# volcengine/veScale

Hardware: AMD Instinct MI355X
Metric: tokens/sec (whole node) Llama-3-8B veScale-FSDP (higher is better)
Workload: dtype bf16; 1 GPU; model=llama3_8b, global_batch=4, seq_len=8192, parallelism=fsdp1, activation_checkpointing=False, hipgraph=True

## Files before the change

### vescale_amd/ops/csrc/attention_bwd.hip

```cpp
#include "common.h"

#define FA_D 128
#define FA_BLK 64
#define FA_THREADS 256
#define FA_PAD 8

typedef float fa_floatx4 __attribute__((ext_vector_type(4)));
typedef short fa_shortx8 __attribute__((ext_vector_type(8)));

extern "C" __global__ void __launch_bounds__(256)
fa_bwd_preprocess(const unsigned short* __restrict__ dout,
                  const unsigned short* __restrict__ o,
                  float* __restrict__ delta, int64_t rows) {
  const int sub = threadIdx.x & 15;
  int64_t row = (int64_t)blockIdx.x * 16 + (threadIdx.x >> 4);
  const int64_t stride = (int64_t)gridDim.x * 16;
  for (; row < rows; row += stride) {
    const unsigned short* pd = dout + row * FA_D + sub * 8;
    const unsigned short* po = o + row * FA_D + sub * 8;
    fa_shortx8 a = *reinterpret_cast<const fa_shortx8*>(pd);
    fa_shortx8 b = *reinterpret_cast<const fa_shortx8*>(po);
    float s = 0.f;
#pragma unroll
    for (int j = 0; j < 8; ++j)
      s += bf16_to_f32((unsigned short)a[j]) * bf16_to_f32((unsigned short)b[j]);
#pragma unroll
    for (int off = 8; off >= 1; off >>= 1)
      s += __shfl_xor(s, off, 64);
    if (sub == 0) delta[row] = s;
  }
}

#define ROWS_N (FA_BLK + FA_PAD)
#define ROWS_D (FA_D + FA_PAD)

DEV void stage_rows(const unsigned short* g, unsigned short* lds_t, int tid) {
#pragma unroll
  for (int j = 0; j < 4; ++j) {
    int e = (tid + j * FA_THREADS) * 8;
    int r = e / FA_D, c = e % FA_D;
    *reinterpret_cast<fa_shortx8*>(lds_t + r * ROWS_D + c) =
        *reinterpret_cast<const fa_shortx8*>(g + r * FA_D + c);
  }
}

DEV void stage_rows_t(const unsigned short* g, unsigned short* lds_t, int tid) {
#pragma unroll
  for (int j = 0; j < 4; ++j) {
    int e = (tid + j * FA_THREADS) * 8;
    int r = e / FA_D, c = e % FA_D;
    fa_shortx8 v = *reinterpret_cast<const fa_shortx8*>(g + r * FA_D + c);
#pragma unroll
    for (int x = 0; x < 8; ++x) lds_t[(c + x) * ROWS_N + r] = (unsigned short)v[x];
  }
}

DEV fa_shortx8 frag(const unsigned short* t, int stride, int rf, int kc, int lane) {
  int row = rf * 16 + (lane & 15);
  int col = kc * 32 + (lane >> 4) * 8;
  return *reinterpret_cast<const fa_shortx8*>(t + row * stride + col);
}

extern "C" __global__ void __launch_bounds__(FA_THREADS)
fa_bwd_dkdv(const unsigned short* __restrict__ q,
            const unsigned short* __restrict__ k,
            const unsigned short* __restrict__ v,
            const unsigned short* __restrict__ dout,
            const float* __restrict__ lse,
            const float* __restrict__ delta,
            unsigned short* __restrict__ dk_part,
            unsigned short* __restrict__ dv_part,
            int B, int Hq, int Hkv, int S, float scale) {
  __shared__ unsigned short lq[FA_D * ROWS_N];
  __shared__ unsigned short ldo[FA_D * ROWS_N];
  __shared__ unsigned short lpt[FA_BLK * ROWS_N];
  __shared__ unsigned short lds_t[FA_BLK * ROWS_N];
  __shared__ float lse_s[FA_BLK];
  __shared__ float dlt_s[FA_BLK];

  const int tid = threadIdx.x;
  const int lane = tid & 63;
  const int wave = tid >> 6;
  const int jkv = blockIdx.x;
  const int h = blockIdx.y;
  const int b = blockIdx.z;
  const int hkv = h / (Hq / Hkv);

  const int64_t qbase = (((int64_t)b * Hq + h) * S) * FA_D;
  const int64_t kbase = (((int64_t)b * Hkv + hkv) * S) * FA_D;
  const int64_t lbase = ((int64_t)b * Hq + h) * S;

  fa_shortx8 kfrag[4], vfrag[4];
  {
    const unsigned short* kg = k + kbase + (int64_t)(jkv * FA_BLK) * FA_D;
    const unsigned short* vg = v + kbase + (int64_t)(jkv * FA_BLK) * FA_D;
    int row = wave * 16 + (lane & 15);
#pragma unroll
    for (int kc = 0; kc < 4; ++kc) {
      int col = kc * 32 + (lane >> 4) * 8;
      kfrag[kc] = *reinterpret_cast<const fa_shortx8*>(kg + row * FA_D + col);
      vfrag[kc] = *reinterpret_cast<const fa_shortx8*>(vg + row * FA_D + col);
    }
  }

  fa_floatx4 accK[8], accV[8];
#pragma unroll
  for (int i = 0; i < 8; ++i) {
    accK[i] = (fa_floatx4){0.f, 0.f, 0.f, 0.f};
    accV[i] = (fa_floatx4){0.f, 0.f, 0.f, 0.f};
  }

  const int n_qtiles = S / FA_BLK;
  for (int iq = jkv; iq < n_qtiles; ++iq) {
    const unsigned short* qg = q + qbase + (int64_t)(iq * FA_BLK) * FA_D;
    const unsigned short* dog = dout + qbase + (int64_t)(iq * FA_BLK) * FA_D;
    fa_shortx8 regq[4], regdo[4];
#pragma unroll
    for (int j = 0; j < 4; ++j) {
      int e = (tid + j * FA_THREADS) * 8;
      int r = e / FA_D, c = e % FA_D;
      regq[j] = *reinterpret_cast<const fa_shortx8*>(qg + r * FA_D + c);
      regdo[j] = *reinterpret_cast<const fa_shortx8*>(dog + r * FA_D + c);
      *reinterpret_cast<fa_shortx8*>(lq + r * ROWS_D + c) = regq[j];
      *reinterpret_cast<fa_shortx8*>(ldo + r * ROWS_D + c) = regdo[j];
    }
    if (tid < FA_BLK) {
      lse_s[tid] = lse[lbase + iq * FA_BLK + tid];
      dlt_s[tid] = delta[lbase + iq * FA_BLK + tid];
    }
    __syncthreads();

    fa_floatx4 st[4], dpt[4];
#pragma unroll
    for (int f = 0; f < 4; ++f) {
      st[f] = (fa_floatx4){0.f, 0.f, 0.f, 0.f};
      dpt[f] = (fa_floatx4){0.f, 0.f, 0.f, 0.f};
    }
#pragma unroll
    for (int kc = 0; kc < 4; ++kc) {
#pragma unroll
      for (int f = 0; f < 4; ++f) {
        fa_shortx8 bq = frag(lq, ROWS_D, f, kc, lane);
        st[f] = __builtin_amdgcn_mfma_f32_16x16x32_bf16(kfrag[kc], bq, st[f], 0, 0, 0);
        fa_shortx8 bd = frag(ldo, ROWS_D, f, kc, lane);
        dpt[f] = __builtin_amdgcn_mfma_f32_16x16x32_bf16(vfrag[kc], bd, dpt[f], 0, 0, 0);
      }
    }

    const int kvrow = jkv * FA_BLK + wave * 16 + 4 * (lane >> 4);
    __syncthreads();
#pragma unroll
    for (int f = 0; f < 4; ++f) {
      int qcol = f * 16 + (lane & 15);
      float l = lse_s[qcol];
      float dl = dlt_s[qcol];
      int qidx = iq * FA_BLK + qcol;
#pragma unroll
      for (int r = 0; r < 4; ++r) {
        bool valid = qidx >= (kvrow + r);
        float p = valid ? __expf(st[f][r] * scale - l) : 0.f;
        float ds = p * (dpt[f][r] - dl) * scale;
        int row = wave * 16 + 4 * (lane >> 4) + r;
        lpt[row * ROWS_N + qcol] = f32_to_bf16(p);
        lds_t[row * ROWS_N + qcol] = f32_to_bf16(ds);
      }
    }
#pragma unroll
    for (int j = 0; j < 4; ++j) {
      int e = (tid + j * FA_THREADS) * 8;
      int r = e / FA_D, c = e % FA_D;
#pragma unroll
      for (int x = 0; x < 8; ++x) {
        lq[(c + x) * ROWS_N + r] = (unsigned short)regq[j][x];
        ldo[(c + x) * ROWS_N + r] = (unsigned short)regdo[j][x];
      }
    }
    __syncthreads();

#pragma unroll
    for (int kc = 0; kc < 2; ++kc) {
      fa_shortx8 xp = frag(lpt, ROWS_N, wave, kc, lane);
      fa_shortx8 xs = frag(lds_t, ROWS_N, wave, kc, lane);
#pragma unroll
      for (int f = 0; f < 8; ++f) {
        fa_shortx8 yd = frag(ldo, ROWS_N, f, kc, lane);
        accV[f] = __builtin_amdgcn_mfma_f32_16x16x32_bf16(xp, yd, accV[f], 0, 0, 0);
        fa_shortx8 yq = frag(lq, ROWS_N, f, kc, lane);
        accK[f] = __builtin_amdgcn_mfma_f32_16x16x32_bf16(xs, yq, accK[f], 0, 0, 0);
      }
    }
    __syncthreads();
  }

  unsigned short* dkg = dk_part + qbase + (int64_t)(jkv * FA_BLK) * FA_D;
  unsigned short* dvg = dv_part + qbase + (int64_t)(jkv * FA_BLK) * FA_D;
#pragma unroll
  for (int f = 0; f < 8; ++f) {
    int col = f * 16 + (lane & 15);
#pragma unroll
    for (int r = 0; r < 4; ++r) {
      int row = wave * 16 + 4 * (lane >> 4) + r;
      dkg[(int64_t)row * FA_D + col] = f32_to_bf16(accK[f][r]);
      dvg[(int64_t)row * FA_D + col] = f32_to_bf16(accV[f][r]);
    }
  }
}

extern "C" __global__ void __launch_bounds__(FA_THREADS)
fa_bwd_dq(const unsigned short* __restrict__ q,
          const unsigned short* __restrict__ k,
          const unsigned short* __restrict__ v,
          const unsigned short* __restrict__ dout,
          const float* __restrict__ lse,
          const float* __restrict__ delta,
          unsigned short* __restrict__ dq,
          int B, int Hq, int Hkv, int S, float scale) {
  __shared__ unsigned short lk[FA_D * ROWS_N];
  __shared__ unsigned short lv[FA_BLK * ROWS_D];
  __shared__ unsigned short lds_s[FA_BLK * ROWS_N];

  const int tid = threadIdx.x;
  const int lane = tid & 63;
  const int wave = tid >> 6;
  const int iq = blockIdx.x;
  const int h = blockIdx.y;
  const int b = blockIdx.z;
  const int hkv = h / (Hq / Hkv);

  const int64_t qbase = (((int64_t)b * Hq + h) * S) * FA_D;
  const int64_t kbase = (((int64_t)b * Hkv + hkv) * S) * FA_D;
  const int64_t lbase = ((int64_t)b * Hq + h) * S;

  fa_shortx8 qfrag[4], dofrag[4];
  {
    const unsigned short* qg = q + qbase + (int64_t)(iq * FA_BLK) * FA_D;
    const unsigned short* dog = dout + qbase + (int64_t)(iq * FA_BLK) * FA_D;
    int row = wave * 16 + (lane & 15);
#pragma unroll
    for (int kc = 0; kc < 4; ++kc) {
      int col = kc * 32 + (lane >> 4) * 8;
      qfrag[kc] = *reinterpret_cast<const fa_shortx8*>(qg + row * FA_D + col);
      dofrag[kc] = *reinterpret_cast<const fa_shortx8*>(dog + row * FA_D + col);
    }
  }
  float lse_r[4], dlt_r[4];
#pragma unroll
  for (int r = 0; r < 4; ++r) {
    int row = iq * FA_BLK + wave * 16 + 4 * (lane >> 4) + r;
    lse_r[r] = lse[lbase + row];
    dlt_r[r] = delta[lbase + row];
  }

  fa_floatx4 accQ[8];
#pragma unroll
  for (int i = 0; i < 8; ++i) accQ[i] = (fa_floatx4){0.f, 0.f, 0.f, 0.f};

  for (int jkv = 0; jkv <= iq; ++jkv) {
    const unsigned short* kg = k + kbase + (int64_t)(jkv * FA_BLK) * FA_D;
    const unsigned short* vg = v + kbase + (int64_t)(jkv * FA_BLK) * FA_D;
    fa_shortx8 regk[4];
#pragma unroll
    for (int j = 0; j < 4; ++j) {
      int e = (tid + j * FA_THREADS) * 8;
      int r = e / FA_D, c = e % FA_D;
      regk[j] = *reinterpret_cast<const fa_shortx8*>(kg + r * FA_D + c);
      *reinterpret_cast<fa_shortx8*>(lk + r * ROWS_D + c) = regk[j];
      *reinterpret_cast<fa_shortx8*>(lv + r * ROWS_D + c) =
          *reinterpret_cast<const fa_shortx8*>(vg + r * FA_D + c);
    }
    __syncthreads();

    fa_floatx4 sacc[4], dp[4];
#pragma unroll
    for (int f = 0; f < 4; ++f) {
      sacc[f] = (fa_floatx4){0.f, 0.f, 0.f, 0.f};
      dp[f] = (fa_floatx4){0.f, 0.f, 0.f, 0.f};
    }
#pragma unroll
    for (int kc = 0; kc < 4; ++kc) {
#pragma unroll
      for (int f = 0; f < 4; ++f) {
        fa_shortx8 yk = frag(lk, ROWS_D, f, kc, lane);
        sacc[f] = __builtin_amdgcn_mfma_f32_16x16x32_bf16(qfrag[kc], yk, sacc[f], 0, 0, 0);
        fa_shortx8 yv = frag(lv, ROWS_D, f, kc, lane);
        dp[f] = __builtin_amdgcn_mfma_f32_16x16x32_bf16(dofrag[kc], yv, dp[f], 0, 0, 0);
      }
    }
    __syncthreads();

    const int qrow0 = iq * FA_BLK + wave * 16 + 4 * (lane >> 4);
#pragma unroll
    for (int f = 0; f < 4; ++f) {
      int kvcol = jkv * FA_BLK + f * 16 + (lane & 15);
#pragma unroll
      for (int r = 0; r < 4; ++r) {
        bool valid = (qrow0 + r) >= kvcol;
        float p = valid ? __expf(sacc[f][r] * scale - lse_r[r]) : 0.f;
        float ds = p * (dp[f][r] - dlt_r[r]) * scale;
        int row = wave * 16 + 4 * (lane >> 4) + r;
        lds_s[row * ROWS_N + f * 16 + (lane & 15)] = f32_to_bf16(ds);
      }
    }
#pragma unroll
    for (int j = 0; j < 4; ++j) {
      int e = (tid + j * FA_THREADS) * 8;
      int r = e / FA_D, c = e % FA_D;
#pragma unroll
      for (int x = 0; x < 8; ++x) lk[(c + x) * ROWS_N + r] = (unsigned short)regk[j][x];
    }
    __syncthreads();

#pragma unroll
    for (int kc = 0; kc < 2; ++kc) {
      fa_shortx8 xs = frag(lds_s, ROWS_N, wave, kc, lane);
#pragma unroll
      for (int f = 0; f < 8; ++f) {
        fa_shortx8 yk = frag(lk, ROWS_N, f, kc, lane);
        accQ[f] = __builtin_amdgcn_mfma_f32_16x16x32_bf16(xs, yk, accQ[f], 0, 0, 0);
      }
    }
    __syncthreads();
  }

  unsigned short* dqg = dq + qbase + (int64_t)(iq * FA_BLK) * FA_D;
#pragma unroll
  for (int f = 0; f < 8; ++f) {
    int col = f * 16 + (lane & 15);
#pragma unroll
    for (int r = 0; r < 4; ++r) {
      int row = wave * 16 + 4 * (lane >> 4) + r;
      dqg[(int64_t)row * FA_D + col] = f32_to_bf16(accQ[f][r]);
    }
  }
}

extern "C" __global__ void __launch_bounds__(256)
fa_bwd_reduce_gqa(const unsigned short* __restrict__ part,
                  unsigned short* __restrict__ out,
                  int B, int Hq, int Hkv, int64_t SD) {
  int group = Hq / Hkv;
  int64_t total = (int64_t)B * Hkv * SD;
  int64_t i0 = (int64_t)(blockIdx.x * 256 + threadIdx.x) * 8;
  int64_t stride = (int64_t)gridDim.x * 256 * 8;
  for (int64_t i = i0; i < total; i += stride) {
    int64_t bh = i / SD;
    int64_t off = i % SD;
    int64_t b = bh / Hkv;
    int64_t hk = bh % Hkv;
    float acc[8] = {0, 0, 0, 0, 0, 0, 0, 0};
#pragma unroll 4
    for (int g = 0; g < group; ++g) {
      const unsigned short* p =
          part + ((b * Hq + hk * group + g) * SD) + off;
      fa_shortx8 v = *reinterpret_cast<const fa_shortx8*>(p);
#pragma unroll
      for (int j = 0; j < 8; ++j) acc[j] += bf16_to_f32((unsigned short)v[j]);
    }
    fa_shortx8 o;
#pragma unroll
    for (int j = 0; j < 8; ++j) o[j] = (short)f32_to_bf16(acc[j]);
    *reinterpret_cast<fa_shortx8*>(out + i) = o;
  }
}
```

### vescale_amd/ops/csrc/attention_bwd2.hip

```cpp
#include "fa32_common.h"

#define FB_D FF_D
#define FB_OWN 32
#define FB_WAVES 8
#define FB_TILE (FB_OWN * FB_WAVES)
#define FB_OTH 64
#define FB_THREADS (FB_WAVES * 64)

extern "C" __global__ void __launch_bounds__(FB_THREADS, 2)
fa2_dq_bf16(const unsigned short* __restrict__ q,
            const unsigned short* __restrict__ k,
            const unsigned short* __restrict__ v,
            const unsigned short* __restrict__ dout,
            const float* __restrict__ lse,
            const float* __restrict__ delta,
            unsigned short* __restrict__ dq,
            int B, int Hq, int Hkv, int S, float scale) {
  __shared__ unsigned short lk[FB_OTH * FB_D];
  __shared__ unsigned short lv[FB_OTH * FB_D];
  __shared__ unsigned short ldo[FB_TILE * FB_D];

  const ff_ctx c = ff_prologue(Hq, Hkv, S);
  const int tid = c.tid, wave = c.wave, l31 = c.l31, half = c.half;
  const int qt = c.tile;
  const int64_t qbase = c.qbase, kbase = c.kbase;
  const int q0 = qt * FB_TILE + wave * FB_OWN;
  const int my_q = q0 + l31;
  const float scale2 = scale * FF_LOG2E;

  const int64_t lrow = c.rbase + my_q;
  const float lse2 = lse[lrow] * FF_LOG2E;
  const float dlt = delta[lrow];

  ff_shortx8 qf[8];
  ff_row_frags(q + qbase + (int64_t)my_q * FB_D, qf, half);
  ff_stage<FB_TILE, FB_THREADS>(dout + qbase + (int64_t)qt * FB_TILE * FB_D, ldo, tid);

  ff_floatx16 dqacc[4];
#pragma unroll
  for (int i = 0; i < 4; ++i) dqacc[i] = (ff_floatx16)(0.f);

  const int last_kv = min((qt + 1) * (FB_TILE / FB_OTH), S / FB_OTH);
  const unsigned short* kg = k + kbase;
  const unsigned short* vg = v + kbase;

  for (int jkv = 0; jkv < last_kv; ++jkv) {
    const int kv0 = jkv * FB_OTH;
    const bool active = (kv0 <= q0 + FB_OWN - 1);
    const bool need_mask = (kv0 + FB_OTH - 1 > q0);
    __syncthreads();
    ff_stage<FB_OTH, FB_THREADS>(kg + (int64_t)kv0 * FB_D, lk, tid);
    ff_stage<FB_OTH, FB_THREADS>(vg + (int64_t)kv0 * FB_D, lv, tid);
    __syncthreads();

    if (active) {
      ff_floatx16 st[2], dp[2];
#pragma unroll
      for (int s2 = 0; s2 < 2; ++s2) {
        st[s2] = (ff_floatx16)(0.f);
        dp[s2] = (ff_floatx16)(0.f);
      }
#pragma unroll
      for (int s2 = 0; s2 < 2; ++s2)
#pragma unroll
        for (int ks = 0; ks < 8; ++ks) {
          ff_shortx8 kfr = ff_afrag(lk, s2, ks, l31, half);
          st[s2] = __builtin_amdgcn_mfma_f32_32x32x16_bf16(kfr, qf[ks], st[s2], 0, 0, 0);
          ff_shortx8 vfr = ff_afrag(lv, s2, ks, l31, half);
          ff_shortx8 dof = ff_bfrag(ldo, wave * FB_OWN + l31, ks, half);
          dp[s2] = __builtin_amdgcn_mfma_f32_32x32x16_bf16(vfr, dof, dp[s2], 0, 0, 0);
        }
#pragma unroll
      for (int s2 = 0; s2 < 2; ++s2)
#pragma unroll
        for (int r = 0; r < 16; ++r) {
          int kv = ff_drow(kv0 + s2 * 32, r, half);
          float x = st[s2][r] * scale2 - lse2;
          if (need_mask && kv > my_q) x = -INFINITY;
          float p = __builtin_amdgcn_exp2f(x);
          st[s2][r] = p * (dp[s2][r] - dlt);
        }
      ff_shortx8 pb[4];
      ff_relayout(st, pb, half);
#pragma unroll
      for (int ds = 0; ds < 4; ++ds) {
        ff_shortx4 t[4][2];
        ff_tr_read8(lk, ds, tid, l31, half, t);
#pragma unroll
        for (int ks = 0; ks < 4; ++ks)
          dqacc[ds] = __builtin_amdgcn_mfma_f32_32x32x16_bf16(
              ff_cat(t[ks][0], t[ks][1]), pb[ks], dqacc[ds], 0, 0, 0);
      }
    }
  }

  ff_store_row(dq + qbase + (int64_t)my_q * FB_D, dqacc, scale, half);
}

template <bool DK>
DEV void fa2_dv_dk_t(const unsigned short* __restrict__ q,
                     const unsigned short* __restrict__ k,
                     const unsigned short* __restrict__ v,
                     const unsigned short* __restrict__ dout,
                     const float* __restrict__ lse,
                     const float* __restrict__ delta,
                     unsigned short* __restrict__ out_part,
                     int Hq, int Hkv, int S, float scale) {
  __shared__ unsigned short lq[FB_OTH * FB_D];
  __shared__ unsigned short ldo[FB_OTH * FB_D];
  __shared__ float llse[FB_OTH];
  __shared__ float ldelta[FB_OTH];

  const ff_ctx c = ff_prologue(Hq, Hkv, S);
  const int tid = c.tid, wave = c.wave, l31 = c.l31, half = c.half;
  const int64_t qbase = c.qbase, kbase = c.kbase;
  const int kvB = c.tile * FB_TILE;
  const int kv0w = kvB + wave * FB_OWN;
  const int my_kv = kv0w + l31;
  const float scale2 = scale * FF_LOG2E;

  ff_shortx8 kf[8], vf[DK ? 8 : 1];
  {
    const unsigned short* kg = k + kbase + (int64_t)my_kv * FB_D;
    const unsigned short* vg = DK ? v + kbase + (int64_t)my_kv * FB_D : nullptr;
#pragma unroll
    for (int ks = 0; ks < 8; ++ks) {
      kf[ks] = ff_row_frag(kg, ks, half);
      if constexpr (DK) vf[ks] = ff_row_frag(vg, ks, half);
    }
  }

  ff_floatx16 acc[4];
#pragma unroll
  for (int i = 0; i < 4; ++i) acc[i] = (ff_floatx16)(0.f);

  const int jq0 = kvB / FB_OTH;
  const int n_jq = S / FB_OTH;
  const float* lseg = lse + c.rbase;
  const float* dltg = DK ? delta + c.rbase : nullptr;

  for (int jq = jq0; jq < n_jq; ++jq) {
    const int qt0 = jq * FB_OTH;
    const bool active = (qt0 + FB_OTH - 1 >= kv0w);
    const bool need_mask = (qt0 < kv0w + FB_OWN - 1);
    __syncthreads();
    ff_stage<FB_OTH, FB_THREADS>(q + qbase + (int64_t)qt0 * FB_D, lq, tid);
    ff_stage<FB_OTH, FB_THREADS>(dout + qbase + (int64_t)qt0 * FB_D, ldo, tid);
    if (tid < FB_OTH) {
      llse[tid] = lseg[qt0 + tid] * FF_LOG2E;
      if constexpr (DK) ldelta[tid] = dltg[qt0 + tid];
    }
    __syncthreads();

    if (active) {
      ff_floatx16 st[2], dp[DK ? 2 : 1];
#pragma unroll
      for (int s2 = 0; s2 < 2; ++s2) {
        st[s2] = (ff_floatx16)(0.f);
        if constexpr (DK) dp[s2] = (ff_floatx16)(0.f);
      }
#pragma unroll
      for (int s2 = 0; s2 < 2; ++s2)
#pragma unroll
        for (int ks = 0; ks < 8; ++ks) {
          ff_shortx8 qfr = ff_afrag(lq, s2, ks, l31, half);
          st[s2] = __builtin_amdgcn_mfma_f32_32x32x16_bf16(qfr, kf[ks], st[s2], 0, 0, 0);
          if constexpr (DK) {
            ff_shortx8 dofr = ff_afrag(ldo, s2, ks, l31, half);
            dp[s2] = __builtin_amdgcn_mfma_f32_32x32x16_bf16(dofr, vf[ks], dp[s2], 0, 0, 0);
          }
        }
#pragma unroll
      for (int s2 = 0; s2 < 2; ++s2)
#pragma unroll
        for (int r = 0; r < 16; ++r) {
          int qrow = ff_drow(s2 * 32, r, half);
          float x = st[s2][r] * scale2 - llse[qrow];
          if (need_mask && qt0 + qrow < my_kv) x = -INFINITY;
          float p = __builtin_amdgcn_exp2f(x);
          if constexpr (DK) st[s2][r] = p * (dp[s2][r] - ldelta[qrow]);
          else st[s2][r] = p;
        }
      ff_shortx8 pb[4];
      ff_relayout(st, pb, half);
#pragma unroll
      for (int ds = 0; ds < 4; ++ds) {
        ff_shortx4 t[4][2];
        ff_tr_read8(DK ? lq : ldo, ds, tid, l31, half, t);
#pragma unroll
        for (int ks = 0; ks < 4; ++ks)
          acc[ds] = __builtin_amdgcn_mfma_f32_32x32x16_bf16(
              ff_cat(t[ks][0], t[ks][1]), pb[ks], acc[ds], 0, 0, 0);
      }
    }
  }

  unsigned short* og = out_part + qbase + (int64_t)my_kv * FB_D;
  ff_store_row<DK>(og, acc, scale, half);
}

extern "C" __global__ void __launch_bounds__(FB_THREADS, 2)
fa2_dv_bf16(const unsigned short* __restrict__ q,
            const unsigned short* __restrict__ k,
            const unsigned short* __restrict__ dout,
            const float* __restrict__ lse,
            unsigned short* __restrict__ dv_part,
            int B, int Hq, int Hkv, int S, float scale) {
  fa2_dv_dk_t<false>(q, k, nullptr, dout, lse, nullptr, dv_part, Hq, Hkv, S, scale);
}

extern "C" __global__ void __launch_bounds__(FB_THREADS, 2)
fa2_dk_bf16(const unsigned short* __restrict__ q,
            const unsigned short* __restrict__ k,
            const unsigned short* __restrict__ v,
            const unsigned short* __restrict__ dout,
            const float* __restrict__ lse,
            const float* __restrict__ delta,
            unsigned short* __restrict__ dk_part,
            int B, int Hq, int Hkv, int S, float scale) {
  fa2_dv_dk_t<true>(q, k, v, dout, lse, delta, dk_part, Hq, Hkv, S, scale);
}

#define FD_WAVES 4
#define FD_THREADS (FD_WAVES * 64)
#define FD_TILE (FD_WAVES * FB_OWN)

extern "C" __global__ void __launch_bounds__(FD_THREADS, 1)
fa2_dvdk_bf16(const unsigned short* __restrict__ q,
              const unsigned short* __restrict__ k,
              const unsigned short* __restrict__ v,
              const unsigned short* __restrict__ dout,
              const float* __restrict__ lse,
              const float* __restrict__ delta,
              unsigned short* __restrict__ dv_part,
              unsigned short* __restrict__ dk_part,
              int B, int Hq, int Hkv, int S, float scale) {
  __shared__ unsigned short lq[FB_OTH * FB_D];
  __shared__ unsigned short ldo[FB_OTH * FB_D];
  __shared__ unsigned short lk[FD_TILE * FB_D];
  __shared__ unsigned short lv[FD_TILE * FB_D];

  const int tid = threadIdx.x;
  const int lane = tid & 63;
  const int wave = tid >> 6;
  const int l31 = lane & 31;
  const int half = lane >> 5;

  int bx = blockIdx.x, by = blockIdx.y, bz = blockIdx.z;
  ff_xcd_remap(bx, by, bz);
  const int kt = bx;
  const int h = by;
  const int b = bz;
  const int hkv = h / (Hq / Hkv);
  const int64_t qbase = (((int64_t)b * Hq + h) * S) * FB_D;
  const int64_t kbase = (((int64_t)b * Hkv + hkv) * S) * FB_D;
  const int kvB = kt * FD_TILE;
  const int kv0w = kvB + wave * FB_OWN;
  const int my_kv = kv0w + l31;
  const int myrow = wave * FB_OWN + l31;
  const float scale2 = scale * FF_LOG2E;

  {
    const unsigned short* kg = k + kbase + (int64_t)kvB * FB_D;
    const unsigned short* vg = v + kbase + (int64_t)kvB * FB_D;
#pragma unroll
    for (int j = 0; j < FF_STAGE_CHUNKS(FD_TILE, FD_THREADS); ++j) {
      const int e = ff_chunk<FD_THREADS>(j, tid);
      ff_chunk_store(ff_chunk_load(kg, e), lk, e);
      ff_chunk_store(ff_chunk_load(vg, e), lv, e);
    }
  }

  ff_floatx16 dvacc[4], dkacc[4];
#pragma unroll
  for (int i = 0; i < 4; ++i) {
    dvacc[i] = (ff_floatx16)(0.f);
    dkacc[i] = (ff_floatx16)(0.f);
  }

  const int jq0 = kvB / FB_OTH;
  const int n_jq = S / FB_OTH;
  const float* lseg = lse + ((int64_t)b * Hq + h) * S;
  const float* dltg = delta + ((int64_t)b * Hq + h) * S;

  for (int jq = jq0; jq < n_jq; ++jq) {
    const int qt0 = jq * FB_OTH;
    const bool active = (qt0 + FB_OTH - 1 >= kv0w);
    const bool need_mask = (qt0 < kv0w + FB_OWN - 1);
    __syncthreads();
    ff_stage<FB_OTH, FD_THREADS>(q + qbase + (int64_t)qt0 * FB_D, lq, tid);
    ff_stage<FB_OTH, FD_THREADS>(dout + qbase + (int64_t)qt0 * FB_D, ldo, tid);
    const float lse_reg = lseg[qt0 + lane] * FF_LOG2E;
    const float dlt_reg = dltg[qt0 + lane];
    __syncthreads();

    if (active) {
      ff_floatx16 st[2], dp[2];
#pragma unroll
      for (int s2 = 0; s2 < 2; ++s2) {
        st[s2] = (ff_floatx16)(0.f);
        dp[s2] = (ff_floatx16)(0.f);
      }
#pragma unroll
      for (int s2 = 0; s2 < 2; ++s2)
#pragma unroll
        for (int ks = 0; ks < 8; ++ks) {
          ff_shortx8 kfr = ff_bfrag(lk, myrow, ks, half);
          ff_shortx8 qfr = ff_afrag(lq, s2, ks, l31, half);
          st[s2] = __builtin_amdgcn_mfma_f32_32x32x16_bf16(qfr, kfr, st[s2], 0, 0, 0);
          ff_shortx8 vfr = ff_bfrag(lv, myrow, ks, half);
          ff_shortx8 dofr = ff_afrag(ldo, s2, ks, l31, half);
          dp[s2] = __builtin_amdgcn_mfma_f32_32x32x16_bf16(dofr, vfr, dp[s2], 0, 0, 0);
        }
#pragma unroll
      for (int s2 = 0; s2 < 2; ++s2)
#pragma unroll
        for (int r = 0; r < 16; ++r) {
          int qrow = ff_drow(s2 * 32, r, half);
          float l2 = __int_as_float(
              __builtin_amdgcn_ds_bpermute(qrow * 4, __float_as_int(lse_reg)));
          float x = st[s2][r] * scale2 - l2;
          if (need_mask && qt0 + qrow < my_kv) x = -INFINITY;
          st[s2][r] = __builtin_amdgcn_exp2f(x);
        }
      {
        ff_shortx8 pb[4];
        ff_relayout(st, pb, half);
#pragma unroll
        for (int ds = 0; ds < 4; ++ds) {
          ff_shortx4 t[4][2];
          ff_tr_read8(ldo, ds, tid, l31, half, t);
#pragma unroll
          for (int ks = 0; ks < 4; ++ks)
            dvacc[ds] = __builtin_amdgcn_mfma_f32_32x32x16_bf16(
                ff_cat(t[ks][0], t[ks][1]), pb[ks], dvacc[ds], 0, 0, 0);
        }
      }
#pragma unroll
      for (int s2 = 0; s2 < 2; ++s2)
#pragma unroll
        for (int r = 0; r < 16; ++r) {
          int qrow = ff_drow(s2 * 32, r, half);
          float dl = __int_as_float(
              __builtin_amdgcn_ds_bpermute(qrow * 4, __float_as_int(dlt_reg)));
          st[s2][r] = st[s2][r] * (dp[s2][r] - dl);
        }
      {
        ff_shortx8 pb[4];
        ff_relayout(st, pb, half);
#pragma unroll
        for (int ds = 0; ds < 4; ++ds) {
          ff_shortx4 t[4][2];
          ff_tr_read8(lq, ds, tid, l31, half, t);
#pragma unroll
          for (int ks = 0; ks < 4; ++ks)
            dkacc[ds] = __builtin_amdgcn_mfma_f32_32x32x16_bf16(
                ff_cat(t[ks][0], t[ks][1]), pb[ks], dkacc[ds], 0, 0, 0);
        }
      }
    }
  }

  unsigned short* ogv = dv_part + qbase + (int64_t)my_kv * FB_D;
  unsigned short* ogk = dk_part + qbase + (int64_t)my_kv * FB_D;
#pragma unroll
  for (int ds = 0; ds < 4; ++ds)
#pragma unroll
    for (int r = 0; r < 16; ++r) {
      ff_store_elem(ogv, ds, r, half, dvacc[ds][r]);
      ff_store_elem(ogk, ds, r, half, dkacc[ds][r] * scale);
    }
}
```

### vescale_amd/ops/csrc/attention_fwd.hip

```cpp
#include "fa32_common.h"

#define FF_QBLK 32
#define FF_WAVES 4
#define FF_QTILE (FF_QBLK * FF_WAVES)
#define FF_KV 64
#define FF_THREADS (FF_WAVES * 64)
#define FF_CHUNKS FF_STAGE_CHUNKS(FF_KV, FF_THREADS)

template <int MODE>
DEV void fa_fwd_t(const unsigned short* __restrict__ q,
            const unsigned short* __restrict__ k,
            const unsigned short* __restrict__ v,
            unsigned short* __restrict__ out,
            float* __restrict__ lse,
            int B, int Hq, int Hkv, int S, float scale) {
  __shared__ unsigned short lk[2][FF_KV * FF_D];
  __shared__ unsigned short lv[2][FF_KV * FF_D];

  const ff_ctx c = ff_prologue(Hq, Hkv, S);
  const int tid = c.tid, lane = c.lane, l31 = c.l31, half = c.half;
  const int qt = c.tile;
  const int q0 = qt * FF_QTILE + c.wave * FF_QBLK;
  const int my_q = q0 + l31;
  const float scale2 = (MODE == 5) ? scale : scale * FF_LOG2E;

  ff_shortx8 qf[8];
  ff_row_frags(q + c.qbase + (int64_t)my_q * FF_D, qf, half);

  float m_run = -INFINITY;
  float l_run = 0.f;
  ff_floatx16 oacc[4];
#pragma unroll
  for (int i = 0; i < 4; ++i) oacc[i] = (ff_floatx16)(0.f);

  const int n_kv = (qt + 1) * (FF_QTILE / FF_KV);
  const int last_kv = min(n_kv, S / FF_KV);

  const unsigned short* kg = k + c.kbase;
  const unsigned short* vg = v + c.kbase;
  ff_shortx8 kreg[FF_CHUNKS], vreg[FF_CHUNKS];
#pragma unroll
  for (int j = 0; j < FF_CHUNKS; ++j) {
    const int e = ff_chunk<FF_THREADS>(j, tid);
    kreg[j] = ff_chunk_load(kg, e);
    vreg[j] = ff_chunk_load(vg, e);
  }
#pragma unroll
  for (int j = 0; j < FF_CHUNKS; ++j) {
    const int e = ff_chunk<FF_THREADS>(j, tid);
    ff_chunk_store(kreg[j], lk[0], e);
    ff_chunk_store(vreg[j], lv[0], e);
  }
  __syncthreads();

  for (int jkv = 0; jkv < last_kv; ++jkv) {
    const int kv0 = jkv * FF_KV;
    const int buf = jkv & 1;
    const bool have_next = (jkv + 1 < last_kv);
    const bool active = (MODE == 4) || (kv0 <= q0 + FF_QBLK - 1);
    const bool need_mask = (MODE == 4) || (kv0 + FF_KV - 1 > q0);
    if (have_next) {
      const unsigned short* kn = kg + (int64_t)(kv0 + FF_KV) * FF_D;
      const unsigned short* vn = vg + (int64_t)(kv0 + FF_KV) * FF_D;
#pragma unroll
      for (int j = 0; j < FF_CHUNKS; ++j) {
        const int e = ff_chunk<FF_THREADS>(j, tid);
        kreg[j] = ff_chunk_load(kn, e);
        vreg[j] = ff_chunk_load(vn, e);
      }
    }

    if (active) {
    ff_floatx16 st[2];
#pragma unroll
    for (int s2 = 0; s2 < 2; ++s2) st[s2] = (ff_floatx16)(MODE == 3 ? 1e-3f : 0.f);
    if constexpr (MODE != 3)
#pragma unroll
    for (int s2 = 0; s2 < 2; ++s2) {
#pragma unroll
      for (int ks = 0; ks < 8; ++ks) {
        ff_shortx8 kf = ff_afrag(lk[buf], s2, ks, l31, half);
        st[s2] = __builtin_amdgcn_mfma_f32_32x32x16_bf16(kf, qf[ks], st[s2], 0, 0, 0);
      }
    }

    if constexpr (MODE == 1 || MODE == 3) {
      l_run += 1.f; m_run = 0.f;
    } else {
    float pmax = -INFINITY;
    if (need_mask) {
#pragma unroll
      for (int s2 = 0; s2 < 2; ++s2)
#pragma unroll
        for (int r = 0; r < 16; ++r) {
          int kv = ff_drow(kv0 + s2 * 32, r, half);
          float x = (kv <= my_q) ? st[s2][r] * scale2 : -INFINITY;
          st[s2][r] = x;
          pmax = fmaxf(pmax, x);
        }
    } else {
#pragma unroll
      for (int s2 = 0; s2 < 2; ++s2)
#pragma unroll
        for (int r = 0; r < 16; ++r) {
          float x = st[s2][r] * scale2;
          st[s2][r] = x;
          pmax = fmaxf(pmax, x);
        }
    }
    pmax = fmaxf(pmax, __int_as_float(ff_swap_other(__float_as_int(pmax), half)));
    float m_new = fmaxf(m_run, pmax);
    bool dead = false;
    if constexpr (MODE == 4) dead = (m_new == -INFINITY);
    float corr;
    if constexpr (MODE == 5) corr = __expf(m_run - m_new);
    else corr = __builtin_amdgcn_exp2f(m_run - m_new);
    if (dead) { corr = 1.f; m_new = m_run; }
    float psum = 0.f;
#pragma unroll
    for (int s2 = 0; s2 < 2; ++s2)
#pragma unroll
      for (int r = 0; r < 16; ++r) {
        float p;
        if (dead) p = 0.f;
        else if constexpr (MODE == 5) p = (st[s2][r] == -INFINITY) ? 0.f : __expf(st[s2][r] - m_new);
        else p = __builtin_amdgcn_exp2f(st[s2][r] - m_new);
        st[s2][r] = p;
        psum += p;
      }
    psum += __int_as_float(ff_swap_other(__float_as_int(psum), half));
    l_run = l_run * corr + psum;
    m_run = m_new;

#pragma unroll
    for (int ds = 0; ds < 4; ++ds)
#pragma unroll
      for (int r = 0; r < 16; ++r) oacc[ds][r] *= corr;
    }

    if constexpr (MODE == 2) {
#pragma unroll
      for (int r = 0; r < 16; ++r) oacc[0][r] += st[0][r] + st[1][r];
    } else {
    ff_shortx8 pb[4];
    ff_relayout(st, pb, half);
#pragma unroll
    for (int ds = 0; ds < 4; ++ds) {
      ff_shortx4 t[4][2];
      ff_tr_read8(lv[buf], ds, lane, l31, half, t);
#pragma unroll
      for (int ks = 0; ks < 4; ++ks)
        oacc[ds] = __builtin_amdgcn_mfma_f32_32x32x16_bf16(
            ff_cat(t[ks][0], t[ks][1]), pb[ks], oacc[ds], 0, 0, 0);
    }
    }
    }

    if (have_next) {
#pragma unroll
      for (int j = 0; j < FF_CHUNKS; ++j) {
        const int e = ff_chunk<FF_THREADS>(j, tid);
        ff_chunk_store(kreg[j], lk[buf ^ 1], e);
        ff_chunk_store(vreg[j], lv[buf ^ 1], e);
      }
    }
    __syncthreads();
  }

  float inv_l = (l_run > 0.f) ? 1.0f / l_run : 0.f;
  ff_store_row(out + c.qbase + (int64_t)my_q * FF_D, oacc, inv_l, half);
  if (half == 0)
    lse[c.rbase + my_q] = m_run * (MODE == 5 ? 1.0f : FF_LN2) + __logf(l_run);
}

extern "C" __global__ void __launch_bounds__(FF_THREADS, 2)
fa_fwd_bf16(const unsigned short* q, const unsigned short* k,
            const unsigned short* v, unsigned short* out, float* lse,
            int B, int Hq, int Hkv, int S, float scale) {
  fa_fwd_t<0>(q, k, v, out, lse, B, Hq, Hkv, S, scale);
}
extern "C" __global__ void __launch_bounds__(FF_THREADS, 2)
fa_fwd_bf16_ab1(const unsigned short* q, const unsigned short* k,
                const unsigned short* v, unsigned short* out, float* lse,
                int B, int Hq, int Hkv, int S, float scale) {
  fa_fwd_t<1>(q, k, v, out, lse, B, Hq, Hkv, S, scale);
}
extern "C" __global__ void __launch_bounds__(FF_THREADS, 2)
fa_fwd_bf16_ab2(const unsigned short* q, const unsigned short* k,
                const unsigned short* v, unsigned short* out, float* lse,
                int B, int Hq, int Hkv, int S, float scale) {
  fa_fwd_t<2>(q, k, v, out, lse, B, Hq, Hkv, S, scale);
}
extern "C" __global__ void __launch_bounds__(FF_THREADS, 2)
fa_fwd_bf16_ab3(const unsigned short* q, const unsigned short* k,
                const unsigned short* v, unsigned short* out, float* lse,
                int B, int Hq, int Hkv, int S, float scale) {
  fa_fwd_t<3>(q, k, v, out, lse, B, Hq, Hkv, S, scale);
}
extern "C" __global__ void __launch_bounds__(FF_THREADS, 2)
fa_fwd_bf16_ab4(const unsigned short* q, const unsigned short* k,
                const unsigned short* v, unsigned short* out, float* lse,
                int B, int Hq, int Hkv, int S, float scale) {
  fa_fwd_t<4>(q, k, v, out, lse, B, Hq, Hkv, S, scale);
}
extern "C" __global__ void __launch_bounds__(FF_THREADS, 2)
fa_fwd_bf16_ab5(const unsigned short* q, const unsigned short* k,
                const unsigned short* v, unsigned short* out, float* lse,
                int B, int Hq, int Hkv, int S, float scale) {
  fa_fwd_t<5>(q, k, v, out, lse, B, Hq, Hkv, S, scale);
}
```

### vescale_amd/ops/csrc/extension.hip

```cpp
#include <torch/extension.h>
#include <ATen/cuda/CUDAContext.h>
#include <c10/cuda/CUDAException.h>
#include <c10/cuda/CUDAGuard.h>

#include "rmsnorm.hip"
#include "rope.hip"
#include "rope_qkv.hip"
#include "swiglu.hip"
#include "adamw.hip"
#include "cross_entropy.hip"
#include "philox_random.hip"
#include "gemm.hip"
#include "gemm8.hip"
#include "attention_bwd.hip"
#include "attention_fwd.hip"
#include "attention_bwd2.hip"
#include "attention_gen.hip"

#include <climits>
#include <sstream>
#include <vector>

namespace {

constexpr auto BF16 = at::kBFloat16;
constexpr auto F32 = at::kFloat;
constexpr auto I64 = at::kLong;
using OptTensor = c10::optional<at::Tensor>;

inline const unsigned short* bf16(const at::Tensor& t) {
  return reinterpret_cast<const unsigned short*>(t.const_data_ptr());
}
inline unsigned short* bf16_mut(const at::Tensor& t) {
  return reinterpret_cast<unsigned short*>(t.data_ptr());
}
inline const unsigned short* bf16(const OptTensor& t) {
  return t.has_value() ? bf16(*t) : nullptr;
}
inline float* f32(const OptTensor& t) {
  return t.has_value() ? t->data_ptr<float>() : nullptr;
}

struct Dtypes {
  at::ScalarType a, b;
  Dtypes(at::ScalarType a) : a(a), b(a) {}
  Dtypes(at::ScalarType a, at::ScalarType b) : a(a), b(b) {}
};

struct Shape {
  at::DimVector sizes;
  int64_t numel = -1;
  bool any = true;
  Shape() {}
  Shape(at::IntArrayRef s) : sizes(s.begin(), s.end()), any(false) {}
  Shape(std::initializer_list<int64_t> s) : sizes(s), any(false) {}
  static Shape of_numel(int64_t n) { Shape s; s.numel = n; return s; }
  bool matches(const at::Tensor& t) const {
    if (any) return numel < 0 || t.numel() == numel;
    if (t.dim() != (int64_t)sizes.size()) return false;
    for (int64_t i = 0; i < t.dim(); ++i)
      if (sizes[i] >= 0 && t.size(i) != sizes[i]) return false;
    return true;
  }
};

class Binding {
 public:
  Binding(const char* fn, const char* first_name, const at::Tensor& first)
      : fn(fn), first_name_(first_name), dev_(first.device()) {
    if (first.is_cuda()) guard_.set_device(dev_);
  }

  void arg(const char* name, const at::Tensor& t, Dtypes dt, const Shape& shape = {}) const {
    if (t.device() == dev_ && t.is_contiguous() &&
        (t.scalar_type() == dt.a || t.scalar_type() == dt.b) && shape.matches(t))
      return;
    std::ostringstream want;
    want << "device=" << dev_ << (dev_.is_cuda() ? "" : " (must be a GPU)")
         << " dtype=" << c10::toString(dt.a);
    if (dt.b != dt.a) want << "|" << c10::toString(dt.b);
    if (!shape.any) want << " sizes=" << at::IntArrayRef(shape.sizes);
    if (shape.numel >= 0) want << " numel=" << shape.numel;
    TORCH_CHECK(false, fn, ": argument '", name, "' expected ", want.str(),
                " contiguous=true; got device=", t.device(), " dtype=",
                c10::toString(t.scalar_type()), " sizes=", t.sizes(), " numel=",
                t.numel(), " contiguous=", t.is_contiguous() ? "true" : "false");
  }
  void arg(const char* name, const OptTensor& t, Dtypes dt, const Shape& shape = {}) const {
    if (t.has_value()) arg(name, *t, dt, shape);
  }

  int64_t last_dim(const char* what, const at::Tensor& t, int mult) const {
    int64_t n = t.dim() >= 1 ? t.size(-1) : 0;
    TORCH_CHECK(n > 0 && n % mult == 0, fn, ": ", what, " = ", n,
                " must be a positive multiple of ", mult);
    return n;
  }

  void rope_span(const at::Tensor& table, int64_t pos_offset, int64_t S, int64_t D) const {
    TORCH_CHECK(D > 0 && D % 2 == 0, fn, ": head dim D = ", D, " must be even");
    TORCH_CHECK(pos_offset >= 0, fn, ": pos_offset = ", pos_offset, " must be >= 0");
    TORCH_CHECK(table.dim() == 3 && pos_offset + S <= table.size(0), fn,
                ": pos_offset + S = ", pos_offset + S, " is past the table, sizes=",
                table.sizes());
  }

  template <typename... KArgs, typename... Args>
  void launch(void (*kernel)(KArgs...), dim3 grid, dim3 block, Args&&... args) const {
    TORCH_CHECK(dev_.is_cuda(), fn, ": argument '", first_name_,
                "' expected device=a GPU; got device=", dev_);
    TORCH_CHECK(grid.x > 0 && grid.y > 0 && grid.z > 0, fn, ": zero grid dimension (",
                grid.x, ",", grid.y, ",", grid.z, "); return before launching when there is no work");
    hipLaunchKernelGGL(kernel, grid, block, 0,
                       (hipStream_t)at::cuda::getCurrentCUDAStream().stream(),
                       std::forward<Args>(args)...);
    C10_CUDA_KERNEL_LAUNCH_CHECK();
  }

  const char* const fn;

 private:
  const char* first_name_;
  c10::Device dev_;
  at::cuda::OptionalCUDAGuard guard_;
};

}

#include "probes.hip"

namespace {

std::vector<at::Tensor> rmsnorm_fwd(at::Tensor x, at::Tensor w, double eps) {
  Binding b("rmsnorm_fwd", "x", x);
  int hidden = (int)b.last_dim("hidden (x.size(-1))", x, 8);
  b.arg("x", x, BF16);
  b.arg("w", w, BF16, {hidden});
  int64_t rows = x.numel() / hidden;
  auto out = at::empty_like(x);
  auto rrms = at::empty({rows}, x.options().dtype(F32));
  if (rows == 0) return {out, rrms};
  b.launch(rmsnorm_fwd_bf16, (int)std::min<int64_t>(rows, 2048), 256, bf16(x), bf16(w),
           bf16_mut(out), rrms.data_ptr<float>(), rows, hidden, (float)eps);
  return {out, rrms};
}

std::vector<at::Tensor> rmsnorm_bwd(at::Tensor dy, at::Tensor x, at::Tensor w,
                                    at::Tensor rrms, OptTensor dres) {
  Binding b("rmsnorm_bwd", "dy", dy);
  int hidden = (int)b.last_dim("hidden (dy.size(-1))", dy, 8);
  TORCH_CHECK(hidden <= 8192, "rmsnorm_bwd supports hidden <= 8192, got ", hidden);
  int64_t rows = dy.numel() / hidden;
  b.arg("dy", dy, BF16);
  b.arg("x", x, BF16, dy.sizes());
  b.arg("w", w, BF16, {hidden});
  b.arg("rrms", rrms, F32, {rows});
  b.arg("dres", dres, BF16, dy.sizes());
  auto dx = at::empty_like(x);
  if (rows == 0) return {dx, at::zeros({hidden}, x.options().dtype(F32))};
  int grid = (int)std::min<int64_t>(rows, 1024);
  auto dw_part = at::empty({grid, hidden}, x.options().dtype(F32));
  b.launch(rmsnorm_bwd_bf16, grid, 256, bf16(dy), bf16(x), bf16(w),
           rrms.data_ptr<float>(), bf16(dres), bf16_mut(dx), dw_part.data_ptr<float>(),
           rows, hidden);
  return {dx, dw_part.sum(0)};
}

std::vector<at::Tensor> rmsnorm_res_fwd(at::Tensor x, OptTensor res, at::Tensor w,
                                        double eps) {
  Binding b("rmsnorm_res_fwd", "x", x);
  int hidden = (int)b.last_dim("hidden (x.size(-1))", x, 8);
  b.arg("x", x, BF16);
  b.arg("res", res, BF16, x.sizes());
  b.arg("w", w, BF16, {hidden});
  int64_t rows = x.numel() / hidden;
  auto out = at::empty_like(x);
  auto res_out = at::empty_like(x);
  auto rrms = at::empty({rows}, x.options().dtype(F32));
  if (rows == 0) return {out, res_out, rrms};
  b.launch(rmsnorm_res_fwd_bf16, (int)std::min<int64_t>(rows, 2048), 256, bf16(x),
           bf16(res), bf16(w), bf16_mut(out), bf16_mut(res_out), rrms.data_ptr<float>(),
           rows, hidden, (float)eps);
  return {out, res_out, rrms};
}

at::Tensor rope(at::Tensor x, at::Tensor table, int64_t pos_offset, bool backward,
                bool inplace) {
  Binding b("rope", "x", x);
  TORCH_CHECK(x.dim() == 4, "rope: x must be [B,S,H,D], got sizes=", x.sizes());
  int B = (int)x.size(0), S = (int)x.size(1), H = (int)x.size(2), D = (int)x.size(3);
  b.rope_span(table, pos_offset, S, D);
  b.arg("x", x, BF16);
  b.arg("table", table, F32, {-1, D / 2, 2});
  auto out = inplace ? x : at::empty_like(x);
  int64_t n_tokens = (int64_t)B * S * H;
  int64_t pairs = n_tokens * (D / 2);
  b.launch(rope_fwd_bf16, grid_for(pairs / 2, 256), 256, bf16(x), bf16_mut(out),
           table.data_ptr<float>(), n_tokens, H, S, D, (int)pos_offset,
           backward ? 1 : 0);
  return out;
}

int64_t rope_qkv_check(const Binding& b, const at::Tensor& table, int64_t B, int64_t S,
                       int64_t Hq, int64_t Hkv, int64_t D, int64_t pos_offset) {
  TORCH_CHECK(B >= 0 && S >= 0 && Hq >= 0 && Hkv >= 0 && D <= INT_MAX &&
                  S <= INT_MAX && Hq <= INT_MAX && Hkv <= INT_MAX,
              b.fn, ": B, S, Hq, Hkv must be >= 0 and fit int");
  b.rope_span(table, pos_offset, S, D);
  return B * S * (Hq + 2 * Hkv) * (D / 2);
}

std::vector<at::Tensor> rope_qkv_fwd(at::Tensor qkv, at::Tensor table, int64_t B,
                                     int64_t S, int64_t Hq, int64_t Hkv, int64_t D,
                                     int64_t pos_offset) {
  Binding b("rope_qkv_fwd", "qkv", qkv);
  int64_t total = rope_qkv_check(b, table, B, S, Hq, Hkv, D, pos_offset);
  b.arg("qkv", qkv, BF16, Shape::of_numel(total * 2));
  b.arg("table", table, F32, {-1, D / 2, 2});
  auto opt = qkv.options();
  auto q = at::empty({B, Hq, S, D}, opt);
  auto k = at::empty({B, Hkv, S, D}, opt);
  auto v = at::empty({B, Hkv, S, D}, opt);
  b.launch(rope_qkv_fwd_bf16, grid_for(total, 256), 256, bf16(qkv), bf16_mut(q),
           bf16_mut(k), bf16_mut(v), table.data_ptr<float>(), B * S, (int)S, (int)Hq,
           (int)Hkv, (int)D, (int)pos_offset);
  return {q, k, v};
}

at::Tensor rope_qkv_bwd(at::Tensor dq, at::Tensor dk, at::Tensor dv, at::Tensor table,
                        int64_t B, int64_t S, int64_t Hq, int64_t Hkv, int64_t D,
                        int64_t pos_offset) {
  Binding b("rope_qkv_bwd", "dq", dq);
  int64_t total = rope_qkv_check(b, table, B, S, Hq, Hkv, D, pos_offset);
  b.arg("dq", dq, BF16, {B, Hq, S, D});
  b.arg("dk", dk, BF16, {B, Hkv, S, D});
  b.arg("dv", dv, BF16, {B, Hkv, S, D});
  b.arg("table", table, F32, {-1, D / 2, 2});
  auto dqkv = at::empty({B, S, (Hq + 2 * Hkv) * D}, dq.options());
  b.launch(rope_qkv_bwd_bf16, grid_for(total, 256), 256, bf16(dq), bf16(dk), bf16(dv),
           bf16_mut(dqkv), table.data_ptr<float>(), B * S, (int)S, (int)Hq, (int)Hkv,
           (int)D, (int)pos_offset);
  return dqkv;
}

at::Tensor swiglu_fwd(at::Tensor gate, at::Tensor up) {
  Binding b("swiglu_fwd", "gate", gate);
  b.arg("gate", gate, BF16);
  b.arg("up", up, BF16, gate.sizes());
  auto out = at::empty_like(gate);
  int64_t n = gate.numel();
  b.launch(swiglu_fwd_bf16, grid_for(n / 8, 256), 256, bf16(gate), bf16(up),
           bf16_mut(out), n);
  return out;
}

std::vector<at::Tensor> swiglu_bwd(at::Tensor dy, at::Tensor gate, at::Tensor up) {
  Binding b("swiglu_bwd", "dy", dy);
  b.arg("dy", dy, BF16);
  b.arg("gate", gate, BF16, dy.sizes());
  b.arg("up", up, BF16, dy.sizes());
  auto dgate = at::empty_like(gate);
  auto dup = at::empty_like(up);
  int64_t n = gate.numel();
  b.launch(swiglu_bwd_bf16, grid_for(n / 8, 256), 256, bf16(dy), bf16(gate), bf16(up),
           bf16_mut(dgate), bf16_mut(dup), n);
  return {dgate, dup};
}

at::Tensor swiglu_packed_fwd(at::Tensor gu) {
  Binding b("swiglu_packed_fwd", "gu", gu);
  int F = (int)b.last_dim("packed ffn dim F2 (gu.size(-1))", gu, 16) / 2;
  b.arg("gu", gu, BF16);
  int64_t rows = gu.numel() / (2 * F);
  auto sizes = gu.sizes().vec();
  sizes.back() = F;
  auto out = at::empty(sizes, gu.options());
  b.launch(swiglu_packed_fwd_bf16, grid_for(rows * (F / 8), 256), 256, bf16(gu),
           bf16_mut(out), rows, F);
  return out;
}

at::Tensor swiglu_packed_bwd(at::Tensor dy, at::Tensor gu) {
  Binding b("swiglu_packed_bwd", "dy", dy);
  int F = (int)b.last_dim("packed ffn dim F2 (gu.size(-1))", gu, 16) / 2;
  auto sizes = gu.sizes().vec();
  sizes.back() = F;
  b.arg("dy", dy, BF16, at::IntArrayRef(sizes));
  b.arg("gu", gu, BF16);
  int64_t rows = gu.numel() / (2 * F);
  auto dgu = at::empty_like(gu);
  b.launch(swiglu_packed_bwd_bf16, grid_for(rows * (F / 8), 256), 256, bf16(dy),
           bf16(gu), bf16_mut(dgu), rows, F);
  return dgu;
}


void ce_vp_check(const Binding& b, int64_t n, int64_t vocab_start, int64_t vocab_total) {
  TORCH_CHECK(vocab_total >= -1, b.fn, ": vocab_total = ", vocab_total,
              " must be >= 0, or -1 for the dense kernel");
  TORCH_CHECK(vocab_start >= 0, b.fn, ": vocab_start = ", vocab_start, " must be >= 0");
  TORCH_CHECK(vocab_total == -1 ? vocab_start == 0 : vocab_start <= vocab_total - n, b.fn,
              ": vocab_start + n = ", vocab_start, " + ", n,
              " is past vocab_total = ", vocab_total);
}

std::vector<at::Tensor> ce_fwd(at::Tensor logits, at::Tensor target,
                               int64_t ignore_index, int64_t vocab_start,
                               int64_t vocab_total) {
  Binding b("ce_fwd", "logits", logits);
  int vocab = (int)b.last_dim("vocab (logits.size(-1))", logits, 8);
  ce_vp_check(b, vocab, vocab_start, vocab_total);
  int64_t rows = logits.numel() / vocab;
  b.arg("logits", logits, BF16);
  b.arg("target", target, I64, Shape::of_numel(rows));
  auto loss = at::empty({rows}, logits.options().dtype(F32));
  auto lse = at::empty({rows}, logits.options().dtype(F32));
  if (rows == 0) return {loss, lse};
  int grid = (int)std::min<int64_t>(rows, 2048);
  if (vocab_total < 0)
    b.launch(ce_fwd_bf16, grid, 256, bf16(logits), target.data_ptr<int64_t>(),
             loss.data_ptr<float>(), lse.data_ptr<float>(), rows, vocab, ignore_index);
  else
    b.launch(ce_vp_fwd_bf16, grid, 256, bf16(logits), target.data_ptr<int64_t>(),
             loss.data_ptr<float>(), lse.data_ptr<float>(), rows, vocab, vocab_start,
             ignore_index);
  return {loss, lse};
}

at::Tensor ce_bwd(at::Tensor logits, at::Tensor target, at::Tensor lse,
                  at::Tensor dloss, int64_t ignore_index, bool inplace,
                  int64_t vocab_start, int64_t vocab_total) {
  Binding b("ce_bwd", "logits", logits);
  int vocab = (int)b.last_dim("vocab (logits.size(-1))", logits, 8);
  ce_vp_check(b, vocab, vocab_start, vocab_total);
  int64_t rows = logits.numel() / vocab;
  b.arg("logits", logits, BF16);
  b.arg("target", target, I64, Shape::of_numel(rows));
  b.arg("lse", lse, F32, {rows});
  b.arg("dloss", dloss, F32, {rows});
  auto dlogits = inplace ? logits : at::empty_like(logits);
  if (rows == 0) return dlogits;
  int grid = (int)std::min<int64_t>(rows, 2048);
  if (vocab_total < 0)
    b.launch(ce_bwd_bf16, grid, 256, bf16(logits), bf16_mut(dlogits),
             target.data_ptr<int64_t>(), lse.data_ptr<float>(), dloss.data_ptr<float>(),
             rows, vocab, ignore_index);
  else
    b.launch(ce_vp_bwd_bf16, grid, 256, bf16(logits), bf16_mut(dlogits),
             target.data_ptr<int64_t>(), lse.data_ptr<float>(), dloss.data_ptr<float>(),
             rows, vocab, vocab_start, ignore_index);
  return dlogits;
}

void adamw_step(at::Tensor param, OptTensor master, at::Tensor grad, at::Tensor m,
                at::Tensor v, double lr, double beta1, double beta2, double eps,
                double weight_decay, int64_t step, double grad_scale,
                OptTensor clip_scale) {
  Binding b("adamw_step", "param", param);
  TORCH_CHECK(step >= 1, "adamw_step: step = ", step, " must be >= 1");
  int64_t n = param.numel();
  b.arg("param", param, BF16);
  b.arg("master", master, F32, Shape::of_numel(n));
  b.arg("grad", grad, {BF16, F32}, Shape::of_numel(n));
  b.arg("m", m, F32, Shape::of_numel(n));
  b.arg("v", v, F32, Shape::of_numel(n));
  b.arg("clip_scale", clip_scale, F32);
  TORCH_CHECK(!clip_scale.has_value() || clip_scale->numel() >= 1,
              "adamw_step: argument 'clip_scale' needs at least one element");
  float bc1 = 1.f - powf((float)beta1, (float)step);
  float bc2 = 1.f - powf((float)beta2, (float)step);
  bool gbf = grad.scalar_type() == BF16;
  b.launch(adamw_flat_bf16, grid_for(n / 8, 256), 256, bf16_mut(param), f32(master),
           gbf ? bf16(grad) : nullptr, gbf ? nullptr : grad.data_ptr<float>(),
           m.data_ptr<float>(), v.data_ptr<float>(), n, (float)lr, (float)beta1,
           (float)beta2, (float)eps, (float)weight_decay, bc1, bc2, (float)grad_scale,
           f32(clip_scale));
}

at::Tensor l2norm_sq(at::Tensor x) {
  Binding b("l2norm_sq", "x", x);
  b.arg("x", x, {BF16, F32});
  int64_t n = x.numel();
  if (n == 0) return at::zeros({1}, x.options().dtype(F32));
  int grid = grid_for(n / 8, 256);
  auto part = at::empty({grid}, x.options().dtype(F32));
  bool xbf = x.scalar_type() == BF16;
  b.launch(l2norm_sq_flat, grid, 256, xbf ? bf16(x) : nullptr,
           xbf ? nullptr : x.data_ptr<float>(), part.data_ptr<float>(), n);
  return part.sum(0, true);
}

void scale_(at::Tensor x, OptTensor scale_t, double scale_c) {
  Binding b("scale_", "x", x);
  b.arg("x", x, {BF16, F32});
  b.arg("scale_t", scale_t, F32);
  TORCH_CHECK(!scale_t.has_value() || scale_t->numel() >= 1,
              "scale_: argument 'scale_t' needs at least one element");
  int64_t n = x.numel();
  if (n == 0) return;
  bool xbf = x.scalar_type() == BF16;
  b.launch(scale_flat, grid_for(n / 8, 256), 256, xbf ? bf16_mut(x) : nullptr,
           xbf ? nullptr : x.data_ptr<float>(), f32(scale_t), (float)scale_c, n);
}

void gemm_check(const Binding& b, const at::Tensor& a, const at::Tensor& bm, int BM,
                int BN, int BK) {
  TORCH_CHECK(a.dim() == 2 && bm.dim() == 2, b.fn, ": a and b must be 2-D, got a sizes=",
              a.sizes(), " b sizes=", bm.sizes());
  int64_t M = a.size(0), K = a.size(1), N = bm.size(0);
  TORCH_CHECK(M >= 1 && N >= 1 && K >= 1 && M <= INT_MAX && N <= INT_MAX && K <= INT_MAX,
              b.fn, ": M, N, K must be >= 1 and fit int");
  TORCH_CHECK(M % BM == 0 && N % BN == 0 && K % BK == 0, b.fn,
              " tile divisibility violated: requires M % ", BM, " == 0, N % ", BN,
              " == 0 and K % ", BK, " == 0");
  b.arg("a", a, BF16);
  b.arg("b", bm, BF16, {N, K});
}

at::Tensor gemm_tn(at::Tensor a, at::Tensor b, int64_t variant) {
  Binding bd("gemm_tn", "a", a);
  TORCH_CHECK(variant >= 0 && variant <= 4, "gemm_tn: variant = ", variant,
              " must be in 0..4");
  int BM = variant == 1 ? 128 : (variant == 3 ? 128 : (variant == 4 ? 512 : 256));
  int BN = variant == 3 ? 128 : 256;
  int BK = variant == 1 ? 64 : 32;
  int threads = variant == 3 ? 256 : (variant == 4 ? 1024 : 512);
  gemm_check(bd, a, b, BM, BN, BK);
  int64_t M = a.size(0), K = a.size(1), N = b.size(0);
  auto c = at::empty({M, N}, a.options());
  decltype(&gemm_tn_bf16_v0) kerns[] = {gemm_tn_bf16_v0, gemm_tn_bf16_v1, gemm_tn_bf16_v2,
                                        gemm_tn_bf16_v3, gemm_tn_bf16_v4};
  bd.launch(kerns[variant], (int)((M / BM) * (N / BN)), threads, bf16(a), bf16(b),
            bf16_mut(c), (int)M, (int)N, (int)K);
  return c;
}

at::Tensor gemm_tn8(at::Tensor a, at::Tensor b, int64_t mode) {
  Binding bd("gemm_tn8", "a", a);
  TORCH_CHECK(mode >= 0 && mode <= 8, "gemm_tn8: mode = ", mode, " must be in 0..8");
  gemm_check(bd, a, b, G8_BM, G8_BN, G8_BK);
  int64_t M = a.size(0), K = a.size(1), N = b.size(0);
  TORCH_CHECK(mode != 5 || (K / 64) % 2 == 0, "mode 5 needs K % 128 == 0");
  TORCH_CHECK((mode != 7 && mode != 8) || ((K / 64) % 2 == 0 && K / 64 >= 4),
              "modes 7/8 need an even K/64 >= 4");
  auto c = at::empty({M, N}, a.options());
  decltype(&gemm8_tn_bf16) kerns[] = {
      gemm8_tn_bf16,        gemm8_tn_bf16_lockstep, gemm8_tn_bf16_rot,
      gemm8_tn_bf16_rot3,   gemm8_tn_bf16_rot3np,   gemm8_tn_bf16_rot3u2,
      gemm8_tn_bf16_rot3ra, gemm8_tn_bf16_rot8,     gemm8_tn_bf16_rot9};
  bd.launch(kerns[mode], dim3((unsigned)(M / 256), (unsigned)(N / 256), 1), G8_THREADS,
            bf16(a), bf16(b), bf16_mut(c), (int)M, (int)N, (int)K);
  return c;
}

struct FaShape { int B, Hq, Hkv, S; };

FaShape fa_check(const Binding& b, int tile, const at::Tensor& q, const at::Tensor& k,
                 const at::Tensor& v, const OptTensor& o = {},
                 const OptTensor& dout = {}, const OptTensor& lse = {}) {
  TORCH_CHECK(q.dim() == 4 && k.dim() == 4, b.fn, ": q, k must be [B,H,S,128], got q sizes=",
              q.sizes(), " k sizes=", k.sizes());
  int64_t B = q.size(0), Hq = q.size(1), S = q.size(2), Hkv = k.size(1);
  TORCH_CHECK(S >= 1 && S % tile == 0 && S <= INT_MAX, b.fn, ": seq = ", S,
              " must be a positive multiple of ", tile);
  TORCH_CHECK(B >= 1 && Hkv >= 1 && Hq >= 1 && Hq % Hkv == 0, b.fn, ": B = ", B,
              " must be >= 1 and Hq = ", Hq, " a positive multiple of Hkv = ", Hkv);
  b.arg("q", q, BF16, {B, Hq, S, FF_D});
  b.arg("k", k, BF16, {B, Hkv, S, FF_D});
  b.arg("v", v, BF16, {B, Hkv, S, FF_D});
  b.arg("o", o, BF16, {B, Hq, S, FF_D});
  b.arg("dout", dout, BF16, {B, Hq, S, FF_D});
  b.arg("lse", lse, F32, {B, Hq, S});
  return {(int)B, (int)Hq, (int)Hkv, (int)S};
}
static_assert(FA_D == FF_D && FB_D == FF_D, "tuned attention kernels share D");

std::vector<at::Tensor> fa_fwd_impl(const Binding& b, int64_t mode, at::Tensor q,
                                    at::Tensor k, at::Tensor v, double scale) {
  FaShape s = fa_check(b, FF_QTILE, q, k, v);
  auto out = at::empty_like(q);
  auto lse = at::empty({s.B, s.Hq, s.S}, q.options().dtype(F32));
  decltype(&fa_fwd_bf16) kerns[] = {fa_fwd_bf16,     fa_fwd_bf16_ab1, fa_fwd_bf16_ab2,
                                    fa_fwd_bf16_ab3, fa_fwd_bf16_ab4, fa_fwd_bf16_ab5};
  b.launch(kerns[mode], dim3(s.S / FF_QTILE, s.Hq, s.B), FF_THREADS, bf16(q), bf16(k), bf16(v),
           bf16_mut(out), lse.data_ptr<float>(), s.B, s.Hq, s.Hkv, s.S, (float)scale);
  return {out, lse};
}

std::vector<at::Tensor> fa_fwd(at::Tensor q, at::Tensor k, at::Tensor v, double scale) {
  return fa_fwd_impl(Binding("fa_fwd", "q", q), 0, q, k, v, scale);
}

std::vector<at::Tensor> fa_fwd_ablate(at::Tensor q, at::Tensor k, at::Tensor v,
                                      double scale, int64_t mode) {
  TORCH_CHECK(mode >= 0 && mode <= 5, "fa_fwd_ablate: mode = ", mode,
              " must be in 0..5");
  return fa_fwd_impl(Binding("fa_fwd_ablate", "q", q), mode, q, k, v, scale);
}

at::Tensor fa_bwd_delta(const Binding& b, const FaShape& s, const at::Tensor& dout,
                        const at::Tensor& o) {
  auto delta = at::empty({s.B, s.Hq, s.S}, o.options().dtype(F32));
  int64_t rows = (int64_t)s.B * s.Hq * s.S;
  b.launch(fa_bwd_preprocess, grid_for(rows, 1, 4096), 256, bf16(dout), bf16(o),
           delta.data_ptr<float>(), rows);
  return delta;
}

at::Tensor fa_bwd_reduce(const Binding& b, const FaShape& s, const at::Tensor& part) {
  if (s.Hkv == s.Hq) return part;
  auto out = at::empty({s.B, s.Hkv, s.S, FF_D}, part.options());
  int64_t SD = (int64_t)s.S * FF_D;
  b.launch(fa_bwd_reduce_gqa, grid_for((int64_t)s.B * s.Hkv * SD / 8, 256), 256,
           bf16(part), bf16_mut(out), s.B, s.Hq, s.Hkv, SD);
  return out;
}

std::vector<at::Tensor> fa_bwd(at::Tensor q, at::Tensor k, at::Tensor v, at::Tensor o,
                               at::Tensor dout, at::Tensor lse, double scale) {
  Binding b("fa_bwd", "q", q);
  FaShape s = fa_check(b, FA_BLK, q, k, v, o, dout, lse);
  auto delta = fa_bwd_delta(b, s, dout, o);
  auto dq = at::empty_like(q);
  auto dk_part = at::empty_like(q);
  auto dv_part = at::empty_like(q);
  dim3 gridkv(s.S / FA_BLK, s.Hq, s.B);
  b.launch(fa_bwd_dkdv, gridkv, FA_THREADS, bf16(q), bf16(k), bf16(v), bf16(dout),
           lse.data_ptr<float>(), delta.data_ptr<float>(), bf16_mut(dk_part),
           bf16_mut(dv_part), s.B, s.Hq, s.Hkv, s.S, (float)scale);
  b.launch(fa_bwd_dq, gridkv, FA_THREADS, bf16(q), bf16(k), bf16(v), bf16(dout),
           lse.data_ptr<float>(), delta.data_ptr<float>(), bf16_mut(dq), s.B, s.Hq,
           s.Hkv, s.S, (float)scale);
  return {dq, fa_bwd_reduce(b, s, dk_part), fa_bwd_reduce(b, s, dv_part)};
}

std::vector<at::Tensor> fa_bwd2(at::Tensor q, at::Tensor k, at::Tensor v, at::Tensor o,
                                at::Tensor dout, at::Tensor lse, double scale,
                                bool fused_dvdk) {
  Binding b("fa_bwd2", "q", q);
  FaShape s = fa_check(b, FB_TILE, q, k, v, o, dout, lse);
  auto delta = fa_bwd_delta(b, s, dout, o);
  auto dq = at::empty_like(q);
  dim3 grid(s.S / FB_TILE, s.Hq, s.B);
  b.launch(fa2_dq_bf16, grid, FB_THREADS, bf16(q), bf16(k), bf16(v), bf16(dout),
           lse.data_ptr<float>(), delta.data_ptr<float>(), bf16_mut(dq), s.B, s.Hq,
           s.Hkv, s.S, (float)scale);
  auto dv_part = at::empty_like(q);
  auto dk_part = at::empty_like(q);
  if (fused_dvdk) {
    b.launch(fa2_dvdk_bf16, dim3(s.S / FD_TILE, s.Hq, s.B), FD_THREADS, bf16(q),
             bf16(k), bf16(v), bf16(dout), lse.data_ptr<float>(),
             delta.data_ptr<float>(), bf16_mut(dv_part), bf16_mut(dk_part), s.B, s.Hq,
             s.Hkv, s.S, (float)scale);
  } else {
    b.launch(fa2_dv_bf16, grid, FB_THREADS, bf16(q), bf16(k), bf16(dout),
             lse.data_ptr<float>(), bf16_mut(dv_part), s.B, s.Hq, s.Hkv, s.S,
             (float)scale);
    b.launch(fa2_dk_bf16, grid, FB_THREADS, bf16(q), bf16(k), bf16(v), bf16(dout),
             lse.data_ptr<float>(), delta.data_ptr<float>(), bf16_mut(dk_part), s.B,
             s.Hq, s.Hkv, s.S, (float)scale);
  }
  return {dq, fa_bwd_reduce(b, s, dk_part), fa_bwd_reduce(b, s, dv_part)};
}

struct FaGenShape { int B, Hq, Hkv, Sq, Sk, D, shift; };

FaGenShape fa_gen_check(const Binding& b, const at::Tensor& q, const at::Tensor& k,
                        const at::Tensor& v, bool causal, int64_t shift) {
  TORCH_CHECK(q.dim() == 4 && k.dim() == 4 && v.dim() == 4,
              b.fn, ": q, k, v must be [B, H, S, D]");
  int64_t D = q.size(3);
  TORCH_CHECK(D == 64 || D == 128, b.fn, ": fa_gen supports head_dim 64 and 128");
  TORCH_CHECK(k.size(1) >= 1 && q.size(1) % k.size(1) == 0,
              b.fn, ": Hq must be a multiple of Hkv");
  TORCH_CHECK(q.size(2) >= 1 && k.size(2) >= 1, b.fn, ": Sq and Sk must be >= 1");
  TORCH_CHECK(q.size(0) >= 1 && q.size(0) <= 65535 && q.size(1) <= 65535,
              b.fn, ": B and Hq must be in [1, 65535]");
  TORCH_CHECK(q.size(2) + k.size(2) < (int64_t)1 << 30, b.fn, ": sequence too long");
  TORCH_CHECK(causal || shift == 0, b.fn, ": shift needs causal");
  b.arg("q", q, BF16);
  b.arg("k", k, BF16, {q.size(0), -1, -1, D});
  b.arg("v", v, BF16, k.sizes());
  int64_t sh = std::max<int64_t>(-q.size(2), std::min<int64_t>(k.size(2), shift));
  return {(int)q.size(0), (int)q.size(1), (int)k.size(1), (int)q.size(2),
          (int)k.size(2), (int)D, (int)sh};
}

#define FA_GEN_KERNEL(kernel, D) ((D) == 64 ? kernel<64> : kernel<128>)

std::vector<at::Tensor> fa_gen_fwd(at::Tensor q, at::Tensor k, at::Tensor v,
                                   double scale, bool causal, int64_t shift) {
  Binding b("fa_gen_fwd", "q", q);
  FaGenShape s = fa_gen_check(b, q, k, v, causal, shift);
  auto out = at::empty_like(q);
  auto lse = at::empty({s.B, s.Hq, s.Sq}, q.options().dtype(F32));
  b.launch(FA_GEN_KERNEL(fa_gen_fwd_kernel, s.D),
           dim3((s.Sq + FG_BLK - 1) / FG_BLK, s.Hq, s.B), FG_THREADS, bf16(q), bf16(k),
           bf16(v), bf16_mut(out), lse.data_ptr<float>(), s.Hq, s.Hkv, s.Sq, s.Sk,
           (float)(scale * 1.4426950408889634), causal ? 1 : 0, s.shift);
  return {out, lse};
}

std::vector<at::Tensor> fa_gen_bwd(at::Tensor q, at::Tensor k, at::Tensor v,
                                   at::Tensor o, at::Tensor dout, at::Tensor lse,
                                   OptTensor dlse, double scale, bool causal,
                                   int64_t shift) {
  Binding b("fa_gen_bwd", "q", q);
  FaGenShape s = fa_gen_check(b, q, k, v, causal, shift);
  b.arg("o", o, BF16, q.sizes());
  b.arg("dout", dout, BF16, q.sizes());
  b.arg("lse", lse, F32, {s.B, s.Hq, s.Sq});
  b.arg("dlse", dlse, F32, {s.B, s.Hq, s.Sq});
  auto delta = at::empty({s.B, s.Hq, s.Sq}, q.options().dtype(F32));
  auto dq = at::empty_like(q);
  auto dk = at::empty_like(k);
  auto dv = at::empty_like(v);
  int64_t rows = (int64_t)s.B * s.Hq * s.Sq;
  b.launch(FA_GEN_KERNEL(fa_gen_preprocess_kernel, s.D),
           grid_for(rows, 256 / (s.D / 8), 4096), 256, bf16(dout), bf16(o),
           lse.data_ptr<float>(), f32(dlse), delta.data_ptr<float>(), rows);
  b.launch(FA_GEN_KERNEL(fa_gen_dkdv_kernel, s.D),
           dim3((s.Sk + FG_BLK - 1) / FG_BLK, s.Hkv, s.B), FG_THREADS, bf16(q), bf16(k),
           bf16(v), bf16(dout), lse.data_ptr<float>(), delta.data_ptr<float>(),
           bf16_mut(dk), bf16_mut(dv), s.Hq, s.Hkv, s.Sq, s.Sk, (float)scale,
           causal ? 1 : 0, s.shift);
  b.launch(FA_GEN_KERNEL(fa_gen_dq_kernel, s.D),
           dim3((s.Sq + FG_BLK - 1) / FG_BLK, s.Hq, s.B), FG_THREADS, bf16(q), bf16(k),
           bf16(v), bf16(dout), lse.data_ptr<float>(), delta.data_ptr<float>(),
           bf16_mut(dq), s.Hq, s.Hkv, s.Sq, s.Sk, (float)scale, causal ? 1 : 0,
           s.shift);
  return {dq, dk, dv};
}

using Dims = std::vector<int64_t>;

ShardDesc make_desc(const char* fn, const Dims& gshape, const Dims& lshape,
                    const Dims& offset, int64_t flat_offset, bool is_flat,
                    int64_t numel) {
  TORCH_CHECK(gshape.size() <= MAXD && lshape.size() == gshape.size() &&
                  offset.size() == gshape.size(),
              fn, ": gshape, lshape, offset must have one length <= ", MAXD,
              ", got ", gshape.size(), ", ", lshape.size(), ", ", offset.size());
  ShardDesc d{};
  d.ndim = (int)gshape.size();
  int64_t prod = 1;
  for (int i = 0; i < d.ndim; ++i) {
    d.gshape[i] = gshape[i];
    d.lshape[i] = lshape[i];
    d.offset[i] = offset[i];
    prod *= lshape[i];
  }
  TORCH_CHECK(prod == numel, fn, ": prod(lshape) = ", prod,
              " must equal the tensor's numel = ", numel);
  d.flat_offset = flat_offset;
  d.is_flat = is_flat ? 1 : 0;
  return d;
}

template <bool NORMAL>
void philox_fill(at::Tensor out, Dims gshape, Dims lshape, Dims offset,
                 int64_t flat_offset, bool is_flat, int64_t seed, int64_t philox_offset,
                 double p0, double p1) {
  Binding b(NORMAL ? "philox_normal_" : "philox_uniform_", "out", out);
  int64_t n = out.numel();
  auto d = make_desc(b.fn, gshape, lshape, offset, flat_offset, is_flat, n);
  b.arg("out", out, {BF16, F32});
  if (out.scalar_type() == BF16)
    b.launch(NORMAL ? philox_normal_bf16 : philox_uniform_bf16, grid_for(n, 256), 256,
             bf16_mut(out), d, n, (uint64_t)seed, (uint64_t)philox_offset, (float)p0,
             (float)p1);
  else
    b.launch(NORMAL ? philox_normal_f32 : philox_uniform_f32, grid_for(n, 256), 256,
             out.data_ptr<float>(), d, n, (uint64_t)seed, (uint64_t)philox_offset,
             (float)p0, (float)p1);
}

std::vector<at::Tensor> philox_dropout(at::Tensor x, Dims gshape, Dims lshape,
                                       Dims offset, int64_t flat_offset, bool is_flat,
                                       int64_t seed, int64_t philox_offset, double p,
                                       bool need_mask) {
  Binding b("philox_dropout", "x", x);
  TORCH_CHECK(p >= 0.0 && p < 1.0, "philox_dropout: p = ", p, " must be in [0, 1)");
  int64_t n = x.numel();
  auto d = make_desc(b.fn, gshape, lshape, offset, flat_offset, is_flat, n);
  b.arg("x", x, BF16);
  auto out = at::empty_like(x);
  at::Tensor mask;
  if (need_mask) mask = at::empty(x.sizes(), x.options().dtype(at::kByte));
  b.launch(philox_dropout_bf16, grid_for(n, 256), 256, bf16(x), bf16_mut(out),
           need_mask ? mask.data_ptr<unsigned char>() : nullptr, d, n, (uint64_t)seed,
           (uint64_t)philox_offset, (float)p);
  if (need_mask) return {out, mask};
  return {out};
}

}

PYBIND11_MODULE(TORCH_EXTENSION_NAME, m) {
  m.def("rmsnorm_fwd", &rmsnorm_fwd);
  m.def("rmsnorm_bwd", &rmsnorm_bwd, pybind11::arg("dy"), pybind11::arg("x"),
        pybind11::arg("w"), pybind11::arg("rrms"),
        pybind11::arg("dres") = pybind11::none());
  m.def("rmsnorm_res_fwd", &rmsnorm_res_fwd);
  m.def("rope", &rope);
  m.def("rope_qkv_fwd", &rope_qkv_fwd);
  m.def("rope_qkv_bwd", &rope_qkv_bwd);
  m.def("swiglu_fwd", &swiglu_fwd);
  m.def("swiglu_bwd", &swiglu_bwd);
  m.def("swiglu_packed_fwd", &swiglu_packed_fwd);
  m.def("swiglu_packed_bwd", &swiglu_packed_bwd);
  m.def("ce_fwd", &ce_fwd, pybind11::arg("logits"), pybind11::arg("target"),
        pybind11::arg("ignore_index"), pybind11::arg("vocab_start") = 0,
        pybind11::arg("vocab_total") = -1);
  m.def("ce_bwd", &ce_bwd, pybind11::arg("logits"), pybind11::arg("target"),
        pybind11::arg("lse"), pybind11::arg("dloss"), pybind11::arg("ignore_index"),
        pybind11::arg("inplace"), pybind11::arg("vocab_start") = 0,
        pybind11::arg("vocab_total") = -1);
  m.def("adamw_step", &adamw_step);
  m.def("l2norm_sq", &l2norm_sq);
  m.def("scale_", &scale_);
  m.def("gemm_tn", &gemm_tn, pybind11::arg("a"), pybind11::arg("b"), pybind11::arg("variant") = 0);
  m.def("gemm_tn8", &gemm_tn8, pybind11::arg("a"), pybind11::arg("b"), pybind11::arg("mode") = 0);
  m.def("fa_bwd", &fa_bwd);
  m.def("fa_bwd2", &fa_bwd2);
  m.def("fa_fwd", &fa_fwd);
  m.def("fa_fwd_ablate", &fa_fwd_ablate);
  m.def("fa_gen_fwd", &fa_gen_fwd, pybind11::arg("q"), pybind11::arg("k"),
        pybind11::arg("v"), pybind11::arg("scale"), pybind11::arg("causal"),
        pybind11::arg("shift"));
  m.def("fa_gen_bwd", &fa_gen_bwd, pybind11::arg("q"), pybind11::arg("k"),
        pybind11::arg("v"), pybind11::arg("o"), pybind11::arg("dout"),
        pybind11::arg("lse"), pybind11::arg("dlse"), pybind11::arg("scale"),
        pybind11::arg("causal"), pybind11::arg("shift"));
  m.def("permlane_probe", &permlane_probe);
  m.def("mfma32_probe", &mfma32_probe);
  m.def("tr_probe", &tr_probe);
  m.def("philox_uniform_", &philox_fill<false>);
  m.def("philox_normal_", &philox_fill<true>);
  m.def("philox_dropout", &philox_dropout);
}
```

### vescale_amd/ops/csrc/fa32_common.h

```cpp
#pragma once
#include "common.h"

#define FF_D 128
#define FF_LOG2E 1.44269504088896340736f
#define FF_LN2 0.69314718055994530942f

typedef float ff_floatx16 __attribute__((ext_vector_type(16)));
typedef short ff_shortx4 __attribute__((ext_vector_type(4)));
typedef short ff_shortx8 __attribute__((ext_vector_type(8)));
typedef int ff_intx4 __attribute__((ext_vector_type(4)));
typedef __attribute__((address_space(3))) const unsigned short* ff_lds_p;

DEV int ff_swap_other(int x, int half) {
  auto r = __builtin_amdgcn_permlane32_swap(x, x, false, false);
  return half ? r[0] : r[1];
}

DEV void ff_xcd_remap(int& bx, int& by, int& bz) {
  int gx = gridDim.x, gy = gridDim.y;
  int nwg = gx * gy * (int)gridDim.z;
  if ((nwg & 7) != 0) return;
  int f = bx + gx * (by + gy * bz);
  f = (f & 7) * (nwg >> 3) + (f >> 3);
  bx = f % gx; f /= gx;
  by = f % gy;
  bz = f / gy;
}

struct ff_ctx {
  int tid, lane, wave;
  int l31, half;
  int tile, h, b;
  int64_t rbase;
  int64_t qbase, kbase;
};
DEV ff_ctx ff_prologue(int Hq, int Hkv, int S) {
  ff_ctx c;
  c.tid = threadIdx.x;
  c.lane = c.tid & 63;
  c.wave = c.tid >> 6;
  c.l31 = c.lane & 31;
  c.half = c.lane >> 5;
  int bx = blockIdx.x, by = blockIdx.y, bz = blockIdx.z;
  ff_xcd_remap(bx, by, bz);
  c.tile = bx;
  c.h = by;
  c.b = bz;
  const int hkv = c.h / (Hq / Hkv);
  c.rbase = ((int64_t)c.b * Hq + c.h) * S;
  c.qbase = c.rbase * FF_D;
  c.kbase = (((int64_t)c.b * Hkv + hkv) * S) * FF_D;
  return c;
}

#define ff_drow(base, r, half) ((base) + ((r) & 3) + 8 * ((r) >> 2) + 4 * (half))

DEV int ff_kswz(int byte_off) {
  int row = byte_off >> 8;
  return byte_off ^ ((row & 7) << 4);
}

#define FF_STAGE_CHUNKS(ROWS, THREADS) ((ROWS) * FF_D / ((THREADS) * 8))
template <int THREADS>
DEV int ff_chunk(int j, int tid) { return (tid + j * THREADS) * 8; }
DEV ff_shortx8 ff_chunk_load(const unsigned short* g, int e) {
  return *reinterpret_cast<const ff_shortx8*>(g + e);
}
DEV void ff_chunk_store(ff_shortx8 v, unsigned short* l, int e) {
  *reinterpret_cast<ff_shortx8*>((char*)l + ff_kswz(e * 2)) = v;
}
template <int ROWS, int THREADS>
DEV void ff_stage(const unsigned short* __restrict__ g, unsigned short* l, int tid) {
#pragma unroll
  for (int j = 0; j < FF_STAGE_CHUNKS(ROWS, THREADS); ++j) {
    const int e = ff_chunk<THREADS>(j, tid);
    ff_chunk_store(ff_chunk_load(g, e), l, e);
  }
}

DEV ff_shortx8 ff_afrag(const unsigned short* l, int s2, int ks, int l31, int half) {
  int byte = ((s2 * 32 + l31) * FF_D + ks * 16 + half * 8) * 2;
  return *reinterpret_cast<const ff_shortx8*>((const char*)l + ff_kswz(byte));
}

DEV ff_shortx8 ff_bfrag(const unsigned short* l, int row, int ks, int half) {
  int byte = (row * FF_D + ks * 16 + half * 8) * 2;
  return *reinterpret_cast<const ff_shortx8*>((const char*)l + ff_kswz(byte));
}

DEV ff_shortx8 ff_row_frag(const unsigned short* __restrict__ row, int ks, int half) {
  return *reinterpret_cast<const ff_shortx8*>(row + ks * 16 + half * 8);
}
DEV void ff_row_frags(const unsigned short* __restrict__ row, ff_shortx8 (&f)[8], int half) {
#pragma unroll
  for (int ks = 0; ks < 8; ++ks) f[ks] = ff_row_frag(row, ks, half);
}

DEV void ff_relayout(const ff_floatx16 st[2], ff_shortx8 pb[4], int half) {
#pragma unroll
  for (int s2 = 0; s2 < 2; ++s2) {
#pragma unroll
    for (int g = 0; g < 2; ++g) {
      unsigned lo0, lo1, hi0, hi1;
      asm volatile("v_cvt_pk_bf16_f32 %0, %1, %2" : "=v"(lo0)
                   : "v"(st[s2][g * 8 + 0]), "v"(st[s2][g * 8 + 1]));
      asm volatile("v_cvt_pk_bf16_f32 %0, %1, %2" : "=v"(lo1)
                   : "v"(st[s2][g * 8 + 2]), "v"(st[s2][g * 8 + 3]));
      asm volatile("v_cvt_pk_bf16_f32 %0, %1, %2" : "=v"(hi0)
                   : "v"(st[s2][g * 8 + 4]), "v"(st[s2][g * 8 + 5]));
      asm volatile("v_cvt_pk_bf16_f32 %0, %1, %2" : "=v"(hi1)
                   : "v"(st[s2][g * 8 + 6]), "v"(st[s2][g * 8 + 7]));
      int p0 = ff_swap_other((int)lo0, half);
      int p1 = ff_swap_other((int)lo1, half);
      int p2 = ff_swap_other((int)hi0, half);
      int p3 = ff_swap_other((int)hi1, half);
      ff_intx4 frag;
      if (half == 0) {
        frag = (ff_intx4){(int)lo0, (int)lo1, p0, p1};
      } else {
        frag = (ff_intx4){p2, p3, (int)hi0, (int)hi1};
      }
      pb[s2 * 2 + g] = *reinterpret_cast<ff_shortx8*>(&frag);
    }
  }
}

DEV void ff_tr_read8(const unsigned short* tile, int ds, int l15, int l31, int half,
                     ff_shortx4 (&t)[4][2]) {
  const int col2 = (ds * 32 + (l31 & 16) + (l15 & 3) * 4) * 2;
  const int row0 = half * 8 + ((l15 & 15) >> 2);
  const int a0 = (row0 * 256 + col2) ^ ((row0 & 7) << 4);
  const int row1 = row0 + 4;
  const int a1 = (row1 * 256 + col2) ^ ((row1 & 7) << 4);
  ff_lds_p b0 = (ff_lds_p)((const char*)tile + a0);
  ff_lds_p b1 = (ff_lds_p)((const char*)tile + a1);
  asm volatile(
      "ds_read_b64_tr_b16 %0, %8 offset:0\n\t"
      "ds_read_b64_tr_b16 %1, %9 offset:0\n\t"
      "ds_read_b64_tr_b16 %2, %8 offset:4096\n\t"
      "ds_read_b64_tr_b16 %3, %9 offset:4096\n\t"
      "ds_read_b64_tr_b16 %4, %8 offset:8192\n\t"
      "ds_read_b64_tr_b16 %5, %9 offset:8192\n\t"
      "ds_read_b64_tr_b16 %6, %8 offset:12288\n\t"
      "ds_read_b64_tr_b16 %7, %9 offset:12288\n\t"
      "s_waitcnt lgkmcnt(0)"
      : "=&v"(t[0][0]), "=&v"(t[0][1]), "=&v"(t[1][0]), "=&v"(t[1][1]),
        "=&v"(t[2][0]), "=&v"(t[2][1]), "=&v"(t[3][0]), "=&v"(t[3][1])
      : "v"(b0), "v"(b1));
}

DEV ff_shortx8 ff_cat(const ff_shortx4 a, const ff_shortx4 b) {
  ff_shortx8 r;
#pragma unroll
  for (int x = 0; x < 4; ++x) { r[x] = a[x]; r[4 + x] = b[x]; }
  return r;
}

DEV void ff_store_elem(unsigned short* __restrict__ row, int ds, int r, int half, float x) {
  row[ff_drow(ds * 32, r, half)] = f32_to_bf16(x);
}
template <bool SCALE = true>
DEV void ff_store_row(unsigned short* __restrict__ row, const ff_floatx16 (&acc)[4],
                      float mul, int half) {
#pragma unroll
  for (int ds = 0; ds < 4; ++ds)
#pragma unroll
    for (int r = 0; r < 16; ++r) {
      if constexpr (SCALE) ff_store_elem(row, ds, r, half, acc[ds][r] * mul);
      else ff_store_elem(row, ds, r, half, acc[ds][r]);
    }
}
```

### vescale_amd/ops/csrc/rmsnorm.hip

```cpp
#include "common.h"

#define BLOCK 256

extern "C" __global__ void __launch_bounds__(BLOCK)
rmsnorm_fwd_bf16(const unsigned short* __restrict__ x,
                 const unsigned short* __restrict__ w,
                 unsigned short* __restrict__ out,
                 float* __restrict__ rrms_out,
                 int64_t n_rows, int hidden, float eps) {
  __shared__ float lds[BLOCK / WAVE];
  const int vec = 8;
  const int per_row_iters = (hidden / vec + BLOCK - 1) / BLOCK;
  for (int64_t row = blockIdx.x; row < n_rows; row += gridDim.x) {
    const unsigned short* xr = x + row * hidden;
    unsigned short* orow = out + row * hidden;
    float ss = 0.f;
    for (int it = 0; it < per_row_iters; ++it) {
      int i = (it * BLOCK + threadIdx.x) * vec;
      if (i < hidden) {
        short8v v = *reinterpret_cast<const short8v*>(xr + i);
#pragma unroll
        for (int j = 0; j < vec; ++j) {
          float f = bf16_to_f32((unsigned short)v[j]);
          ss += f * f;
        }
      }
    }
    float total = block_reduce_sum<BLOCK>(ss, lds);
    float rrms = rsqrtf(total / (float)hidden + eps);
    if (threadIdx.x == 0 && rrms_out) rrms_out[row] = rrms;
    for (int it = 0; it < per_row_iters; ++it) {
      int i = (it * BLOCK + threadIdx.x) * vec;
      if (i < hidden) {
        short8v v = *reinterpret_cast<const short8v*>(xr + i);
        short8v wv = *reinterpret_cast<const short8v*>(w + i);
        short8v o;
#pragma unroll
        for (int j = 0; j < vec; ++j) {
          float f = bf16_to_f32((unsigned short)v[j]);
          float g = bf16_to_f32((unsigned short)wv[j]);
          o[j] = (short)f32_to_bf16(f * rrms * g);
        }
        *reinterpret_cast<short8v*>(orow + i) = o;
      }
    }
  }
}

extern "C" __global__ void __launch_bounds__(BLOCK)
rmsnorm_res_fwd_bf16(const unsigned short* __restrict__ x,
                     const unsigned short* __restrict__ res,
                     const unsigned short* __restrict__ w,
                     unsigned short* __restrict__ out,
                     unsigned short* __restrict__ res_out,
                     float* __restrict__ rrms_out,
                     int64_t n_rows, int hidden, float eps) {
  __shared__ float lds[BLOCK / WAVE];
  const int vec = 8;
  const int per_row_iters = (hidden / vec + BLOCK - 1) / BLOCK;
  for (int64_t row = blockIdx.x; row < n_rows; row += gridDim.x) {
    const unsigned short* xr = x + row * hidden;
    const unsigned short* rr = res ? res + row * hidden : nullptr;
    unsigned short* orow = out + row * hidden;
    unsigned short* rout = res_out + row * hidden;
    float ss = 0.f;
    for (int it = 0; it < per_row_iters; ++it) {
      int i = (it * BLOCK + threadIdx.x) * vec;
      if (i < hidden) {
        short8v v = *reinterpret_cast<const short8v*>(xr + i);
        short8v o;
        if (rr) {
          short8v rv = *reinterpret_cast<const short8v*>(rr + i);
#pragma unroll
          for (int j = 0; j < vec; ++j) {
            float f = bf16_to_f32((unsigned short)v[j]) +
                      bf16_to_f32((unsigned short)rv[j]);
            o[j] = (short)f32_to_bf16(f);
            float fr = bf16_to_f32((unsigned short)o[j]);
            ss += fr * fr;
          }
        } else {
#pragma unroll
          for (int j = 0; j < vec; ++j) {
            float f = bf16_to_f32((unsigned short)v[j]);
            o[j] = (short)v[j];
            ss += f * f;
          }
        }
        *reinterpret_cast<short8v*>(rout + i) = o;
      }
    }
    float total = block_reduce_sum<BLOCK>(ss, lds);
    float rrms = rsqrtf(total / (float)hidden + eps);
    if (threadIdx.x == 0 && rrms_out) rrms_out[row] = rrms;
    for (int it = 0; it < per_row_iters; ++it) {
      int i = (it * BLOCK + threadIdx.x) * vec;
      if (i < hidden) {
        short8v v = *reinterpret_cast<const short8v*>(rout + i);
        short8v wv = *reinterpret_cast<const short8v*>(w + i);
        short8v o;
#pragma unroll
        for (int j = 0; j < vec; ++j) {
          float f = bf16_to_f32((unsigned short)v[j]);
          float g = bf16_to_f32((unsigned short)wv[j]);
          o[j] = (short)f32_to_bf16(f * rrms * g);
        }
        *reinterpret_cast<short8v*>(orow + i) = o;
      }
    }
  }
}

extern "C" __global__ void __launch_bounds__(BLOCK)
rmsnorm_bwd_bf16(const unsigned short* __restrict__ dy,
                 const unsigned short* __restrict__ x,
                 const unsigned short* __restrict__ w,
                 const float* __restrict__ rrms_in,
                 const unsigned short* __restrict__ dres,
                 unsigned short* __restrict__ dx,
                 float* __restrict__ dw_part,
                 int64_t n_rows, int hidden) {
  __shared__ float lds[BLOCK / WAVE];
  const int vec = 8;
  const int per_row_iters = (hidden / vec + BLOCK - 1) / BLOCK;
  float dw_acc[32];
#pragma unroll
  for (int j = 0; j < 32; ++j) dw_acc[j] = 0.f;
  float wreg[32];
  #pragma unroll
  for (int it = 0; it < 4; ++it) {
    int i = (it * BLOCK + threadIdx.x) * vec;
    if (i < hidden) {
      short8v wv = *reinterpret_cast<const short8v*>(w + i);
#pragma unroll
      for (int j = 0; j < vec; ++j) wreg[it * vec + j] = bf16_to_f32((unsigned short)wv[j]);
    }
  }

  for (int64_t row = blockIdx.x; row < n_rows; row += gridDim.x) {
    const unsigned short* dyr = dy + row * hidden;
    const unsigned short* xr = x + row * hidden;
    unsigned short* dxr = dx + row * hidden;
    float rrms = rrms_in[row];
    float dot = 0.f;
    float dyreg[32], xreg[32];
#pragma unroll
    for (int it = 0; it < 4; ++it) {
      int i = (it * BLOCK + threadIdx.x) * vec;
      if (i < hidden) {
        short8v dv = *reinterpret_cast<const short8v*>(dyr + i);
        short8v xv = *reinterpret_cast<const short8v*>(xr + i);
#pragma unroll
        for (int j = 0; j < vec; ++j) {
          float dyf = bf16_to_f32((unsigned short)dv[j]);
          float xf = bf16_to_f32((unsigned short)xv[j]);
          dyreg[it * vec + j] = dyf;
          xreg[it * vec + j] = xf;
          dot += dyf * wreg[it * vec + j] * xf;
        }
      }
    }
    float tdot = block_reduce_sum<BLOCK>(dot, lds);
    float coef = tdot * rrms * rrms * rrms / (float)hidden;
#pragma unroll
    for (int it = 0; it < 4; ++it) {
      int i = (it * BLOCK + threadIdx.x) * vec;
      if (i < hidden) {
        short8v o;
        short8v drv;
        if (dres)
          drv = *reinterpret_cast<const short8v*>(dres + row * hidden + i);
#pragma unroll
        for (int j = 0; j < vec; ++j) {
          float dyf = dyreg[it * vec + j];
          float xf = xreg[it * vec + j];
          float g = rrms * wreg[it * vec + j] * dyf - xf * coef;
          if (dres) g += bf16_to_f32((unsigned short)drv[j]);
          o[j] = (short)f32_to_bf16(g);
          dw_acc[it * vec + j] += dyf * xf * rrms;
        }
        *reinterpret_cast<short8v*>(dxr + i) = o;
      }
    }
  }
  float* dwr = dw_part + (int64_t)blockIdx.x * hidden;
  #pragma unroll
  for (int it = 0; it < 4; ++it) {
    int i = (it * BLOCK + threadIdx.x) * vec;
    if (i < hidden) {
#pragma unroll
      for (int j = 0; j < vec; ++j) dwr[i + j] = dw_acc[it * vec + j];
    }
  }
}
```

### vescale_amd/ops/csrc/rope_qkv.hip

```cpp
#include "common.h"

#define BLOCK 256

extern "C" __global__ void __launch_bounds__(BLOCK)
rope_qkv_fwd_bf16(const unsigned short* __restrict__ qkv,
                  unsigned short* __restrict__ q,
                  unsigned short* __restrict__ k,
                  unsigned short* __restrict__ v,
                  const float* __restrict__ table,
                  int64_t n_tokens, int seq, int Hq, int Hkv, int D,
                  int pos_offset) {
  const int rot = D / 2;
  const int row_in = (Hq + 2 * Hkv) * D;
  const int heads_total = Hq + 2 * Hkv;
  int64_t total = n_tokens * heads_total * rot;
  int64_t i0 = blockIdx.x * BLOCK + threadIdx.x;
  int64_t stride = (int64_t)gridDim.x * BLOCK;
  for (int64_t t = i0; t < total; t += stride) {
    int d = (int)(t % rot);
    int64_t th = t / rot;
    int h = (int)(th % heads_total);
    int64_t tok = th / heads_total;
    int64_t s = tok % seq;
    int64_t b = tok / seq;
    const unsigned short* src = qkv + tok * row_in + (int64_t)h * D;
    float x0 = bf16_to_f32(src[d]);
    float x1 = bf16_to_f32(src[d + rot]);
    unsigned short* dst;
    bool do_rope = true;
    if (h < Hq) {
      dst = q + (((b * Hq + h) * seq) + s) * D;
    } else if (h < Hq + Hkv) {
      dst = k + (((b * Hkv + (h - Hq)) * seq) + s) * D;
    } else {
      dst = v + (((b * Hkv + (h - Hq - Hkv)) * seq) + s) * D;
      do_rope = false;
    }
    if (do_rope) {
      const float* tb = table + ((s + pos_offset) * (int64_t)rot + d) * 2;
      float c = tb[0], sn = tb[1];
      dst[d] = f32_to_bf16(x0 * c - x1 * sn);
      dst[d + rot] = f32_to_bf16(x1 * c + x0 * sn);
    } else {
      dst[d] = f32_to_bf16(x0);
      dst[d + rot] = f32_to_bf16(x1);
    }
  }
}

extern "C" __global__ void __launch_bounds__(BLOCK)
rope_qkv_bwd_bf16(const unsigned short* __restrict__ dq,
                  const unsigned short* __restrict__ dk,
                  const unsigned short* __restrict__ dv,
                  unsigned short* __restrict__ dqkv,
                  const float* __restrict__ table,
                  int64_t n_tokens, int seq, int Hq, int Hkv, int D,
                  int pos_offset) {
  const int rot = D / 2;
  const int row_out = (Hq + 2 * Hkv) * D;
  const int heads_total = Hq + 2 * Hkv;
  int64_t total = n_tokens * heads_total * rot;
  int64_t i0 = blockIdx.x * BLOCK + threadIdx.x;
  int64_t stride = (int64_t)gridDim.x * BLOCK;
  for (int64_t t = i0; t < total; t += stride) {
    int d = (int)(t % rot);
    int64_t th = t / rot;
    int h = (int)(th % heads_total);
    int64_t tok = th / heads_total;
    int64_t s = tok % seq;
    int64_t b = tok / seq;
    const unsigned short* src;
    bool do_rope = true;
    if (h < Hq) {
      src = dq + (((b * Hq + h) * seq) + s) * D;
    } else if (h < Hq + Hkv) {
      src = dk + (((b * Hkv + (h - Hq)) * seq) + s) * D;
    } else {
      src = dv + (((b * Hkv + (h - Hq - Hkv)) * seq) + s) * D;
      do_rope = false;
    }
    float x0 = bf16_to_f32(src[d]);
    float x1 = bf16_to_f32(src[d + rot]);
    unsigned short* dst = dqkv + tok * row_out + (int64_t)h * D;
    if (do_rope) {
      const float* tb = table + ((s + pos_offset) * (int64_t)rot + d) * 2;
      float c = tb[0], sn = -tb[1];
      dst[d] = f32_to_bf16(x0 * c - x1 * sn);
      dst[d + rot] = f32_to_bf16(x1 * c + x0 * sn);
    } else {
      dst[d] = f32_to_bf16(x0);
      dst[d + rot] = f32_to_bf16(x1);
    }
  }
}
```

### vescale_amd/ops/functional.py

```python
from __future__ import annotations

from typing import Optional

import os

import torch


def _ext():
    from . import require_ext

    return require_ext()


def _use_hip(*tensors) -> bool:
    from . import has_ext

    on_gpu = all(t.is_cuda for t in tensors if isinstance(t, torch.Tensor))
    if not on_gpu:
        return False
    if not has_ext():
        from . import require_ext

        require_ext()
    return True


class _RMSNorm(torch.autograd.Function):
    @staticmethod
    def forward(ctx, x: torch.Tensor, weight: torch.Tensor, eps: float):
        if _use_hip(x, weight):
            x2, w2 = x.contiguous(), weight.contiguous()
            out, rrms = _ext().rmsnorm_fwd(x2, w2, eps)
            ctx.save_for_backward(x2, w2, rrms)
            ctx.eps = eps
            ctx.hip = True
            return out
        xf = x.float()
        rrms = torch.rsqrt(xf.pow(2).mean(-1, keepdim=True) + eps)
        out = (xf * rrms * weight.float()).to(x.dtype)
        ctx.save_for_backward(x, weight, rrms.squeeze(-1))
        ctx.eps = eps
        ctx.hip = False
        return out

    @staticmethod
    def backward(ctx, dy: torch.Tensor):
        x, w, rrms = ctx.saved_tensors
        if ctx.hip:
            dx, dw = _ext().rmsnorm_bwd(dy.contiguous(), x, w, rrms)
            return dx, dw.to(w.dtype), None
        xf = x.float()
        dyf = dy.float()
        wf = w.float()
        r = rrms.unsqueeze(-1)
        H = x.shape[-1]
        dot = (dyf * wf * xf).sum(-1, keepdim=True)
        dx = (r * wf * dyf - xf * dot * r.pow(3) / H).to(x.dtype)
        dw = (dyf * xf * r).reshape(-1, H).sum(0).to(w.dtype)
        return dx, dw, None


def rmsnorm(x: torch.Tensor, weight: torch.Tensor, eps: float = 1e-5) -> torch.Tensor:
    return _RMSNorm.apply(x, weight, eps)


def build_rope_table(
    seq_len: int, head_dim: int, theta: float = 500000.0, device="cpu"
) -> torch.Tensor:
    rot = head_dim // 2
    inv = 1.0 / (theta ** (torch.arange(0, rot, dtype=torch.float64, device="cpu") / rot))
    pos = torch.arange(seq_len, dtype=torch.float64, device="cpu")
    ang = torch.outer(pos, inv)
    tab = torch.stack([ang.cos(), ang.sin()], dim=-1).to(torch.float32)
    return tab.to(device)


class _RoPE(torch.autograd.Function):
    @staticmethod
    def forward(ctx, x: torch.Tensor, table: torch.Tensor, pos_offset: int):
        ctx.pos_offset = pos_offset
        if _use_hip(x, table):
            ctx.hip = True
            ctx.save_for_backward(table)
            return _ext().rope(x.contiguous(), table.contiguous(), pos_offset, False, False)
        ctx.hip = False
        ctx.save_for_backward(table)
        return _rope_ref(x, table, pos_offset, False)

    @staticmethod
    def backward(ctx, dy: torch.Tensor):
        (table,) = ctx.saved_tensors
        if ctx.hip:
            return _ext().rope(dy.contiguous(), table.contiguous(), ctx.pos_offset, True, False), None, None
        return _rope_ref(dy, table, ctx.pos_offset, True), None, None


def _rope_ref(x, table, pos_offset, backward):
    B, S, H, D = x.shape
    rot = D // 2
    tb = table[pos_offset : pos_offset + S]
    cos = tb[..., 0].unsqueeze(0).unsqueeze(2)
    sin = tb[..., 1].unsqueeze(0).unsqueeze(2)
    if backward:
        sin = -sin
    xf = x.float()
    x0, x1 = xf[..., :rot], xf[..., rot:]
    o0 = x0 * cos - x1 * sin
    o1 = x1 * cos + x0 * sin
    return torch.cat([o0, o1], dim=-1).to(x.dtype)


class _FusedAddRMSNorm(torch.autograd.Function):

    @staticmethod
    def forward(ctx, x: torch.Tensor, res, weight: torch.Tensor, eps: float):
        ctx.has_res = res is not None
        if _use_hip(x, weight) and (res is None or res.dtype == x.dtype):
            w2 = weight.contiguous()
            out, res_new, rrms = _ext().rmsnorm_res_fwd(
                x.contiguous(), res.contiguous() if res is not None else None,
                w2, eps,
            )
            ctx.save_for_backward(res_new, w2, rrms)
            ctx.hip = True
            return out, res_new
        res_new = x if res is None else (x + res)
        xf = res_new.float()
        rrms = torch.rsqrt(xf.pow(2).mean(-1, keepdim=True) + eps)
        out = (xf * rrms * weight.float()).to(x.dtype)
        ctx.save_for_backward(res_new, weight, rrms.squeeze(-1))
        ctx.hip = False
        return out, res_new

    @staticmethod
    def backward(ctx, dy: torch.Tensor, dres_new):
        res_new, w, rrms = ctx.saved_tensors
        if ctx.hip:
            dx, dw = _ext().rmsnorm_bwd(
                dy.contiguous(), res_new, w, rrms,
                dres_new.contiguous() if dres_new is not None else None,
            )
            dw = dw.to(w.dtype)
        else:
            xf = res_new.float()
            dyf = dy.float()
            r = rrms.unsqueeze(-1)
            wf = w.float()
            h = res_new.shape[-1]
            dot = (dyf * wf * xf).sum(-1, keepdim=True)
            dx = (r * wf * dyf - xf * (dot * r.pow(3) / h)).to(res_new.dtype)
            dw = (dyf * xf * r).reshape(-1, h).sum(0).to(w.dtype)
            if dres_new is not None:
                dx = dx + dres_new
        dres = dx if ctx.has_res else None
        return dx, dres, dw, None


def fused_add_rmsnorm(x, res, weight, eps):
    return _FusedAddRMSNorm.apply(x, res, weight, eps)


def rope_apply(x: torch.Tensor, table: torch.Tensor, pos_offset: int = 0) -> torch.Tensor:
    return _RoPE.apply(x, table, pos_offset)


class _RoPEQKV(torch.autograd.Function):

    @staticmethod
    def forward(ctx, qkv: torch.Tensor, table: torch.Tensor, n_heads: int,
                n_kv_heads: int, head_dim: int, pos_offset: int):
        B, S, _ = qkv.shape
        ctx.dims = (B, S, n_heads, n_kv_heads, head_dim, pos_offset)
        ctx.save_for_backward(table)
        if _use_hip(qkv, table):
            ctx.hip = True
            q, k, v = _ext().rope_qkv_fwd(
                qkv.contiguous(), table.contiguous(), B, S, n_heads, n_kv_heads, head_dim,
                pos_offset,
            )
            return q, k, v
        ctx.hip = False
        d = n_heads * head_dim
        kv = n_kv_heads * head_dim
        q = qkv[..., :d].reshape(B, S, n_heads, head_dim)
        k = qkv[..., d : d + kv].reshape(B, S, n_kv_heads, head_dim)
        v = qkv[..., d + kv :].reshape(B, S, n_kv_heads, head_dim)
        q = _rope_ref(q, table, pos_offset, False)
        k = _rope_ref(k, table, pos_offset, False)
        return (
            q.permute(0, 2, 1, 3).contiguous(),
            k.permute(0, 2, 1, 3).contiguous(),
            v.permute(0, 2, 1, 3).contiguous(),
        )

    @staticmethod
    def backward(ctx, dq, dk, dv):
        (table,) = ctx.saved_tensors
        B, S, Hq, Hkv, D, pos = ctx.dims
        if ctx.hip:
            dqkv = _ext().rope_qkv_bwd(
                dq.contiguous(), dk.contiguous(), dv.contiguous(),
                table.contiguous(), B, S, Hq, Hkv, D, pos,
            )
            return dqkv, None, None, None, None, None
        dq = dq.permute(0, 2, 1, 3)
        dk = dk.permute(0, 2, 1, 3)
        dv = dv.permute(0, 2, 1, 3)
        dqr = _rope_ref(dq, table, pos, True).reshape(B, S, Hq * D)
        dkr = _rope_ref(dk, table, pos, True).reshape(B, S, Hkv * D)
        dvr = dv.reshape(B, S, Hkv * D)
        return torch.cat([dqr, dkr, dvr], dim=-1), None, None, None, None, None


def rope_qkv(qkv: torch.Tensor, table: torch.Tensor, n_heads: int,
             n_kv_heads: int, head_dim: int, pos_offset: int = 0):
    return _RoPEQKV.apply(qkv, table, n_heads, n_kv_heads, head_dim, pos_offset)


class _SwiGLU(torch.autograd.Function):
    @staticmethod
    def forward(ctx, gate: torch.Tensor, up: torch.Tensor):
        if _use_hip(gate, up):
            g = gate.contiguous()
            u = up.contiguous()
            ctx.save_for_backward(g, u)
            ctx.hip = True
            return _ext().swiglu_fwd(g, u)
        ctx.save_for_backward(gate, up)
        ctx.hip = False
        return (torch.nn.functional.silu(gate.float()) * up.float()).to(gate.dtype)

    @staticmethod
    def backward(ctx, dy: torch.Tensor):
        gate, up = ctx.saved_tensors
        if ctx.hip:
            dgate, dup = _ext().swiglu_bwd(dy.contiguous(), gate, up)
            return dgate, dup
        g = gate.float()
        u = up.float()
        d = dy.float()
        sig = torch.sigmoid(g)
        dgate = (d * u * sig * (1 + g * (1 - sig))).to(gate.dtype)
        dup = (d * g * sig).to(up.dtype)
        return dgate, dup


def swiglu(gate: torch.Tensor, up: torch.Tensor) -> torch.Tensor:
    return _SwiGLU.apply(gate, up)


class _SwiGLUPacked(torch.autograd.Function):

    @staticmethod
    def forward(ctx, gu: torch.Tensor):
        if _use_hip(gu):
            g = gu.contiguous()
            ctx.save_for_backward(g)
            ctx.hip = True
            return _ext().swiglu_packed_fwd(g)
        ctx.save_for_backward(gu)
        ctx.hip = False
        F = gu.shape[-1] // 2
        gate, up = gu[..., :F], gu[..., F:]
        return (torch.nn.functional.silu(gate.float()) * up.float()).to(gu.dtype)

    @staticmethod
    def backward(ctx, dy: torch.Tensor):
        (gu,) = ctx.saved_tensors
        if ctx.hip:
            return _ext().swiglu_packed_bwd(dy.contiguous(), gu)
        F = gu.shape[-1] // 2
        g = gu[..., :F].float()
        u = gu[..., F:].float()
        d = dy.float()
        sig = torch.sigmoid(g)
        dgate = d * u * sig * (1 + g * (1 - sig))
        dup = d * g * sig
        return torch.cat([dgate, dup], dim=-1).to(gu.dtype)


def swiglu_packed(gu: torch.Tensor) -> torch.Tensor:
    return _SwiGLUPacked.apply(gu)


class _FusedCE(torch.autograd.Function):
    @staticmethod
    def forward(ctx, logits: torch.Tensor, target: torch.Tensor, ignore_index: int):
        n_tok = (target != ignore_index).sum().clamp(min=1)
        if _use_hip(logits):
            lg, tg = logits.contiguous(), target.contiguous()
            loss, lse = _ext().ce_fwd(lg, tg, ignore_index)
            ctx.save_for_backward(lg, tg, lse, n_tok)
            ctx.ignore_index = ignore_index
            ctx.hip = True
            return loss.sum() / n_tok.to(loss.dtype)
        xf = logits.float()
        lse = torch.logsumexp(xf, dim=-1)
        valid = target != ignore_index
        tgt = target.clamp(min=0)
        xt = xf.gather(-1, tgt.unsqueeze(-1)).squeeze(-1)
        loss = torch.where(valid, lse - xt, torch.zeros_like(lse))
        ctx.save_for_backward(logits, target, lse, n_tok)
        ctx.ignore_index = ignore_index
        ctx.hip = False
        return loss.sum() / n_tok.to(loss.dtype)

    @staticmethod
    def backward(ctx, dloss: torch.Tensor):
        logits, target, lse, n_tok = ctx.saved_tensors
        scale = (dloss / n_tok.to(dloss.dtype)).float()
        if ctx.hip:
            drow = scale.expand(lse.shape[0]).contiguous()
            dlogits = _ext().ce_bwd(
                logits, target, lse, drow, ctx.ignore_index, False
            )
            return dlogits, None, None
        xf = logits.float()
        p = torch.exp(xf - lse.unsqueeze(-1))
        valid = (target != ctx.ignore_index).unsqueeze(-1)
        tgt = target.clamp(min=0)
        p.scatter_add_(
            -1, tgt.unsqueeze(-1), -torch.ones_like(tgt, dtype=p.dtype).unsqueeze(-1)
        )
        d = (p * scale * valid).to(logits.dtype)
        return d, None, None


def fused_cross_entropy(
    logits: torch.Tensor, target: torch.Tensor, ignore_index: int = -100
) -> torch.Tensor:
    return _FusedCE.apply(logits, target, ignore_index)


def _vp_hip(logits_local: torch.Tensor, *others) -> bool:
    return (
        logits_local.dtype == torch.bfloat16
        and logits_local.shape[-1] > 0
        and logits_local.shape[-1] % 8 == 0
        and _use_hip(logits_local, *others)
    )


def _vp_hit(target, vocab_start, n, ignore_index):
    hit = (target != ignore_index) & (target >= vocab_start) & (target < vocab_start + n)
    return hit, torch.where(hit, target - vocab_start, torch.zeros_like(target))


def _vp_check(logits_local, target, vocab_start, vocab_total):
    n = logits_local.shape[-1]
    if logits_local.dim() != 2 or target.shape != logits_local.shape[:1]:
        raise ValueError(
            f"vocab-parallel CE takes logits_local [N, n] and target [N], got "
            f"{tuple(logits_local.shape)} and {tuple(target.shape)}")
    if vocab_start < 0 or vocab_start + n > vocab_total:
        raise ValueError(
            f"shard columns [{vocab_start}, {vocab_start + n}) are not inside "
            f"the vocabulary [0, {vocab_total})")


@torch.no_grad()
def vp_ce_partials(logits_local, target, vocab_start: int, vocab_total: int,
                   ignore_index: int = -100):
    _vp_check(logits_local, target, vocab_start, vocab_total)
    if _vp_hip(logits_local, target):
        picked, lse_local = _ext().ce_fwd(
            logits_local.contiguous(), target.contiguous(), ignore_index,
            vocab_start=vocab_start, vocab_total=vocab_total)
        return picked, lse_local
    xf = logits_local.to(torch.promote_types(logits_local.dtype, torch.float32))
    hit, col = _vp_hit(target, vocab_start, xf.shape[-1], ignore_index)
    xt = xf.gather(-1, col.unsqueeze(-1)).squeeze(-1)
    return torch.where(hit, xt, torch.zeros_like(xt)), torch.logsumexp(xf, dim=-1)


@torch.no_grad()
def vp_ce_grad(logits_local, target, lse, drow, vocab_start: int, vocab_total: int,
               ignore_index: int = -100, inplace: bool = False):
    _vp_check(logits_local, target, vocab_start, vocab_total)
    if _vp_hip(logits_local, target, lse, drow):
        lg = logits_local.contiguous()
        out = _ext().ce_bwd(
            lg, target.contiguous(), lse.float().contiguous(),
            drow.float().contiguous(), ignore_index, inplace,
            vocab_start=vocab_start, vocab_total=vocab_total)
        if inplace and lg is not logits_local:
            logits_local.copy_(out)
            return logits_local
        return out
    xf = logits_local.to(torch.promote_types(logits_local.dtype, torch.float32))
    hit, col = _vp_hit(target, vocab_start, xf.shape[-1], ignore_index)
    p = torch.exp(xf - lse.to(xf.dtype).unsqueeze(-1))
    p.scatter_add_(-1, col.unsqueeze(-1), -hit.to(p.dtype).unsqueeze(-1))
    scale = torch.where(target != ignore_index, drow.to(p.dtype), torch.zeros_like(drow, dtype=p.dtype))
    d = (p * scale.unsqueeze(-1)).to(logits_local.dtype)
    if inplace:
        logits_local.copy_(d)
        return logits_local
    return d


class _VocabParallelCE(torch.autograd.Function):

    @staticmethod
    def forward(ctx, logits_local, target, vocab_start, vocab_total, group,
                ignore_index, reduction):
        picked, lse_local = vp_ce_partials(
            logits_local, target, vocab_start, vocab_total, ignore_index)
        if group is not None and torch.distributed.get_world_size(group) > 1:
            m = lse_local.clone()
            torch.distributed.all_reduce(
                m, op=torch.distributed.ReduceOp.MAX, group=group)
            m = torch.where(m == float("-inf"), torch.zeros_like(m), m)
            both = torch.stack([torch.exp(lse_local - m), picked])
            torch.distributed.all_reduce(both, group=group)
            lse, picked = m + torch.log(both[0]), both[1]
        else:
            lse = lse_local
        valid = target != ignore_index
        rows = torch.where(valid, lse - picked, torch.zeros_like(lse))
        n_tok = valid.sum().clamp(min=1)
        ctx.save_for_backward(logits_local, target, lse, n_tok)
        ctx.args = (vocab_start, vocab_total, ignore_index, reduction)
        if reduction == "none":
            return rows
        return rows.sum() / n_tok.to(rows.dtype)

    @staticmethod
    def backward(ctx, dloss):
        logits_local, target, lse, n_tok = ctx.saved_tensors
        vocab_start, vocab_total, ignore_index, reduction = ctx.args
        if reduction == "none":
            drow = dloss.to(lse.dtype).contiguous()
        else:
            drow = (dloss / n_tok.to(dloss.dtype)).to(lse.dtype).expand(lse.shape[0]).contiguous()
        d = vp_ce_grad(logits_local, target, lse, drow, vocab_start, vocab_total,
                       ignore_index)
        return d, None, None, None, None, None, None


def vocab_parallel_cross_entropy(
    logits_local: torch.Tensor, target: torch.Tensor, vocab_start: int,
    vocab_total: int, group=None, ignore_index: int = -100,
    reduction: str = "mean",
) -> torch.Tensor:
    if reduction not in ("mean", "none"):
        raise ValueError(f"reduction must be 'mean' or 'none', got {reduction!r}")
    return _VocabParallelCE.apply(
        logits_local, target, int(vocab_start), int(vocab_total), group,
        int(ignore_index), reduction)


class _FlashAttention(torch.autograd.Function):

    @staticmethod
    def forward(ctx, q, k, v, scale):
        out, lse = _ext().fa_fwd(q, k, v, scale)
        ctx.save_for_backward(q, k, v, out, lse)
        ctx.scale = scale
        return out

    @staticmethod
    def backward(ctx, dout):
        q, k, v, out, lse = ctx.saved_tensors
        fused = os.environ.get("VESCALE_FA_FUSED_DVDK", "0") == "1"
        dq, dk, dv = _ext().fa_bwd2(
            q, k, v, out, dout.contiguous(), lse, ctx.scale, fused
        )
        return dq, dk, dv, None


def flash_attention_causal(q, k, v):
    import math

    scale = 1.0 / math.sqrt(q.shape[-1])
    if (
        _use_hip(q, k, v)
        and q.shape[-1] == 128
        and q.shape[2] % 256 == 0
        and os.environ.get("VESCALE_FA", "hip") == "hip"
    ):
        return _FlashAttention.apply(
            q.contiguous(), k.contiguous(), v.contiguous(), scale
        )
    return torch.nn.functional.scaled_dot_product_attention(
        q, k, v, is_causal=True, enable_gqa=q.shape[1] != k.shape[1]
    )


def _attention_ref(q, k, v, is_causal, shift, scale, dtype=None):
    if dtype is None:
        dtype = torch.promote_types(q.dtype, torch.float32)
    B, Hq, Sq, D = q.shape
    Hkv, Sk = k.shape[1], k.shape[2]
    qg = q.to(dtype).reshape(B, Hkv, Hq // Hkv, Sq, D)
    s = (qg @ k.to(dtype).unsqueeze(2).transpose(-1, -2)) * scale
    if is_causal:
        i = torch.arange(Sq, device=q.device).unsqueeze(1)
        j = torch.arange(Sk, device=q.device).unsqueeze(0)
        s = s.masked_fill(j > i + shift, float("-inf"))
    m = s.detach().amax(-1, keepdim=True)
    m = torch.where(m == float("-inf"), torch.zeros_like(m), m)
    e = torch.exp(s - m)
    l = e.sum(-1, keepdim=True)
    dead = l == 0
    l1 = torch.where(dead, torch.ones_like(l), l)
    out = (e / l1) @ v.to(dtype).unsqueeze(2)
    lse = torch.where(dead, torch.full_like(l, float("-inf")), m + torch.log(l1))
    lse_dtype = torch.promote_types(q.dtype, torch.float32)
    return (out.reshape(B, Hq, Sq, D).to(q.dtype),
            lse.reshape(B, Hq, Sq).to(lse_dtype))


class _FlashAttentionGen(torch.autograd.Function):

    @staticmethod
    def forward(ctx, q, k, v, scale, causal, shift):
        out, lse = _ext().fa_gen_fwd(q, k, v, scale, causal, shift)
        ctx.save_for_backward(q, k, v, out, lse)
        ctx.args = (scale, causal, shift)
        ctx.set_materialize_grads(False)
        return out, lse

    @staticmethod
    def backward(ctx, dout, dlse):
        q, k, v, out, lse = ctx.saved_tensors
        scale, causal, shift = ctx.args
        dout = torch.zeros_like(out) if dout is None else dout.contiguous()
        if dlse is not None:
            dlse = dlse.float().contiguous()
        dq, dk, dv = _ext().fa_gen_bwd(
            q, k, v, out, dout, lse, dlse, scale, causal, shift
        )
        return dq, dk, dv, None, None, None


def flash_attention(q, k, v, *, is_causal=False, causal_shift=0, scale=None,
                    return_lse=False):
    import math

    if causal_shift != 0 and not is_causal:
        raise ValueError("causal_shift != 0 requires is_causal=True")
    B, Hq, Sq, D = q.shape
    Hkv, Sk = k.shape[1], k.shape[2]
    if scale is None:
        scale = 1.0 / math.sqrt(D)
    hip = (
        os.environ.get("VESCALE_FA", "hip") == "hip"
        and all(t.is_cuda and t.dtype == torch.bfloat16 for t in (q, k, v))
        and D in (64, 128)
        and Hq % Hkv == 0
        and _use_hip(q, k, v)
    )
    if (hip and not return_lse and is_causal and causal_shift == 0
            and Sq == Sk and D == 128 and Sq % 256 == 0):
        return _FlashAttention.apply(
            q.contiguous(), k.contiguous(), v.contiguous(), scale
        )
    if hip:
        out, lse = _FlashAttentionGen.apply(
            q.contiguous(), k.contiguous(), v.contiguous(), float(scale),
            bool(is_causal), int(causal_shift),
        )
    else:
        out, lse = _attention_ref(q, k, v, is_causal, causal_shift, scale)
    return (out, lse) if return_lse else out


@torch.no_grad()
def adamw_step_flat(
    param_bf16: torch.Tensor,
    master_f32: Optional[torch.Tensor],
    grad: torch.Tensor,
    m: torch.Tensor,
    v: torch.Tensor,
    *,
    lr: float,
    beta1: float = 0.9,
    beta2: float = 0.95,
    eps: float = 1e-8,
    weight_decay: float = 0.0,
    step: int = 1,
    grad_scale: float = 1.0,
    clip_scale: Optional[torch.Tensor] = None,
):
    if _use_hip(param_bf16, grad, m, v):
        _ext().adamw_step(
            param_bf16, master_f32, grad, m, v, lr, beta1, beta2, eps,
            weight_decay, step, grad_scale, clip_scale,
        )
        return
    g = grad.float() * grad_scale
    if clip_scale is not None:
        g = g * clip_scale.item()
    p = master_f32 if master_f32 is not None else param_bf16.float()
    p.mul_(1 - lr * weight_decay)
    m.mul_(beta1).add_(g, alpha=1 - beta1)
    v.mul_(beta2).addcmul_(g, g, value=1 - beta2)
    bc1 = 1 - beta1**step
    bc2 = 1 - beta2**step
    denom = (v / bc2).sqrt().add_(eps)
    p.addcdiv_(m, denom, value=-lr / bc1)
    param_bf16.copy_(p.to(param_bf16.dtype))


@torch.no_grad()
def l2norm_sq(x: torch.Tensor) -> torch.Tensor:
    if _use_hip(x):
        return _ext().l2norm_sq(x.contiguous()).squeeze(0)
    return x.float().pow(2).sum()


@torch.no_grad()
def scale_flat_(x: torch.Tensor, scale) -> None:
    if _use_hip(x):
        if isinstance(scale, torch.Tensor):
            _ext().scale_(x, scale.float().contiguous(), 1.0)
        else:
            _ext().scale_(x, None, float(scale))
        return
    if isinstance(scale, torch.Tensor):
        x.mul_(scale.to(x.dtype))
    else:
        x.mul_(scale)


def _gemm_backend() -> str:
    return os.environ.get("VESCALE_GEMM", "blaslt")


def _g8_ok(m: int, n: int, k: int) -> bool:
    return m % 256 == 0 and n % 256 == 0 and k % 64 == 0


class _Linear8(torch.autograd.Function):

    @staticmethod
    def forward(ctx, x: torch.Tensor, w: torch.Tensor):
        ctx.save_for_backward(x, w)
        xs = x.shape
        x2 = x.reshape(-1, xs[-1])
        m, k = x2.shape
        n = w.shape[0]
        if x.is_cuda and x.dtype == torch.bfloat16 and _g8_ok(m, n, k):
            y = _ext().gemm_tn8(x2.contiguous(), w.contiguous(), 4)
        else:
            y = x2 @ w.t()
        return y.reshape(*xs[:-1], n)

    @staticmethod
    def backward(ctx, dy: torch.Tensor):
        x, w = ctx.saved_tensors
        dys = dy.reshape(-1, dy.shape[-1])
        x2 = x.reshape(-1, x.shape[-1])
        m, n = dys.shape
        k = w.shape[1]
        dx = dw = None
        if ctx.needs_input_grad[0]:
            if dy.is_cuda and dy.dtype == torch.bfloat16 and _g8_ok(m, k, n):
                wt = w.t().contiguous()
                dx = _ext().gemm_tn8(dys.contiguous(), wt, 4)
            else:
                dx = dys @ w
            dx = dx.reshape(x.shape)
        if ctx.needs_input_grad[1]:
            dw = dys.t() @ x2
        return dx, dw


def linear(x: torch.Tensor, w: torch.Tensor,
           bias: Optional[torch.Tensor] = None) -> torch.Tensor:
    if _gemm_backend() == "gemm8" and bias is None:
        return _Linear8.apply(x, w)
    return torch.nn.functional.linear(x, w, bias)
```

Before: 18060 tokens/s.

## Emit attention output in BSHD layout, vectorize RoPE, specialize RMSNorm backward

The flash-attention forward now writes its output directly in [B,S,H,D] layout and returns a transposed view, so the downstream transpose/contiguous copy before the output projection goes away. The backward kernels read dout in that layout with strided staging, and the dq grid is reversed so the heaviest causal tiles start first. Separately, RoPE pack/unpack gets an 8-wide vectorized per-token kernel, and RMSNorm backward is templated on iteration count to cut register use for smaller hidden sizes. Strided staging may lower memory coalescing in the backward kernels, and the fused dv/dk path now needs an extra contiguous copy.

```diff
diff --git a/vescale_amd/ops/csrc/attention_bwd.hip b/vescale_amd/ops/csrc/attention_bwd.hip
--- a/vescale_amd/ops/csrc/attention_bwd.hip
+++ b/vescale_amd/ops/csrc/attention_bwd.hip
@@ -11,7 +11,7 @@
 extern "C" __global__ void __launch_bounds__(256)
 fa_bwd_preprocess(const unsigned short* __restrict__ dout,
                   const unsigned short* __restrict__ o,
-                  float* __restrict__ delta, int64_t rows) {
+                  float* __restrict__ delta, int64_t rows, int Hq, int S, int bshd) {
   const int sub = threadIdx.x & 15;
   int64_t row = (int64_t)blockIdx.x * 16 + (threadIdx.x >> 4);
   const int64_t stride = (int64_t)gridDim.x * 16;
@@ -27,7 +27,13 @@
 #pragma unroll
     for (int off = 8; off >= 1; off >>= 1)
       s += __shfl_xor(s, off, 64);
-    if (sub == 0) delta[row] = s;
+    int64_t drow = row;
+    if (bshd) {
+      const unsigned r = (unsigned)row, bs = r / (unsigned)Hq, h = r - bs * (unsigned)Hq;
+      const unsigned bi = bs / (unsigned)S, sq = bs - bi * (unsigned)S;
+      drow = ((int64_t)bi * Hq + h) * S + sq;
+    }
+    if (sub == 0) delta[drow] = s;
   }
 }
 
diff --git a/vescale_amd/ops/csrc/attention_bwd2.hip b/vescale_amd/ops/csrc/attention_bwd2.hip
--- a/vescale_amd/ops/csrc/attention_bwd2.hip
+++ b/vescale_amd/ops/csrc/attention_bwd2.hip
@@ -15,14 +15,14 @@
             const float* __restrict__ lse,
             const float* __restrict__ delta,
             unsigned short* __restrict__ dq,
-            int B, int Hq, int Hkv, int S, float scale) {
+            int B, int Hq, int Hkv, int S, float scale, int bshd) {
   __shared__ unsigned short lk[FB_OTH * FB_D];
   __shared__ unsigned short lv[FB_OTH * FB_D];
   __shared__ unsigned short ldo[FB_TILE * FB_D];
 
   const ff_ctx c = ff_prologue(Hq, Hkv, S);
   const int tid = c.tid, wave = c.wave, l31 = c.l31, half = c.half;
-  const int qt = c.tile;
+  const int qt = (int)gridDim.x - 1 - c.tile;
   const int64_t qbase = c.qbase, kbase = c.kbase;
   const int q0 = qt * FB_TILE + wave * FB_OWN;
   const int my_q = q0 + l31;
@@ -34,7 +34,9 @@
 
   ff_shortx8 qf[8];
   ff_row_frags(q + qbase + (int64_t)my_q * FB_D, qf, half);
-  ff_stage<FB_TILE, FB_THREADS>(dout + qbase + (int64_t)qt * FB_TILE * FB_D, ldo, tid);
+  const ff_rows dorow = ff_o_rows(c, Hq, S, bshd);
+  ff_stage_rows<FB_TILE, FB_THREADS>(
+      dout + dorow.base + (int64_t)qt * FB_TILE * dorow.stride, dorow.stride, ldo, tid);
 
   ff_floatx16 dqacc[4];
 #pragma unroll
@@ -105,7 +107,7 @@
                      const float* __restrict__ lse,
                      const float* __restrict__ delta,
                      unsigned short* __restrict__ out_part,
-                     int Hq, int Hkv, int S, float scale) {
+                     int Hq, int Hkv, int S, float scale, int bshd) {
   __shared__ unsigned short lq[FB_OTH * FB_D];
   __shared__ unsigned short ldo[FB_OTH * FB_D];
   __shared__ float llse[FB_OTH];
@@ -138,6 +140,7 @@
   const int n_jq = S / FB_OTH;
   const float* lseg = lse + c.rbase;
   const float* dltg = DK ? delta + c.rbase : nullptr;
+  const ff_rows dorow = ff_o_rows(c, Hq, S, bshd);
 
   for (int jq = jq0; jq < n_jq; ++jq) {
     const int qt0 = jq * FB_OTH;
@@ -145,7 +148,8 @@
     const bool need_mask = (qt0 < kv0w + FB_OWN - 1);
     __syncthreads();
     ff_stage<FB_OTH, FB_THREADS>(q + qbase + (int64_t)qt0 * FB_D, lq, tid);
-    ff_stage<FB_OTH, FB_THREADS>(dout + qbase + (int64_t)qt0 * FB_D, ldo, tid);
+    ff_stage_rows<FB_OTH, FB_THREADS>(dout + dorow.base + (int64_t)qt0 * dorow.stride,
+                                      dorow.stride, ldo, tid);
     if (tid < FB_OTH) {
       llse[tid] = lseg[qt0 + tid] * FF_LOG2E;
       if constexpr (DK) ldelta[tid] = dltg[qt0 + tid];
@@ -205,8 +209,8 @@
             const unsigned short* __restrict__ dout,
             const float* __restrict__ lse,
             unsigned short* __restrict__ dv_part,
-            int B, int Hq, int Hkv, int S, float scale) {
-  fa2_dv_dk_t<false>(q, k, nullptr, dout, lse, nullptr, dv_part, Hq, Hkv, S, scale);
+            int B, int Hq, int Hkv, int S, float scale, int bshd) {
+  fa2_dv_dk_t<false>(q, k, nullptr, dout, lse, nullptr, dv_part, Hq, Hkv, S, scale, bshd);
 }
 
 extern "C" __global__ void __launch_bounds__(FB_THREADS, 2)
@@ -217,8 +221,8 @@
             const float* __restrict__ lse,
             const float* __restrict__ delta,
             unsigned short* __restrict__ dk_part,
-            int B, int Hq, int Hkv, int S, float scale) {
-  fa2_dv_dk_t<true>(q, k, v, dout, lse, delta, dk_part, Hq, Hkv, S, scale);
+            int B, int Hq, int Hkv, int S, float scale, int bshd) {
+  fa2_dv_dk_t<true>(q, k, v, dout, lse, delta, dk_part, Hq, Hkv, S, scale, bshd);
 }
 
 #define FD_WAVES 4
diff --git a/vescale_amd/ops/csrc/attention_fwd.hip b/vescale_amd/ops/csrc/attention_fwd.hip
--- a/vescale_amd/ops/csrc/attention_fwd.hip
+++ b/vescale_amd/ops/csrc/attention_fwd.hip
@@ -13,7 +13,7 @@
             const unsigned short* __restrict__ v,
             unsigned short* __restrict__ out,
             float* __restrict__ lse,
-            int B, int Hq, int Hkv, int S, float scale) {
+            int B, int Hq, int Hkv, int S, float scale, int out_bshd) {
   __shared__ unsigned short lk[2][FF_KV * FF_D];
   __shared__ unsigned short lv[2][FF_KV * FF_D];
 
@@ -168,7 +168,8 @@
   }
 
   float inv_l = (l_run > 0.f) ? 1.0f / l_run : 0.f;
-  ff_store_row(out + c.qbase + (int64_t)my_q * FF_D, oacc, inv_l, half);
+  const ff_rows orow = ff_o_rows(c, Hq, S, out_bshd);
+  ff_store_row(out + orow.base + (int64_t)my_q * orow.stride, oacc, inv_l, half);
   if (half == 0)
     lse[c.rbase + my_q] = m_run * (MODE == 5 ? 1.0f : FF_LN2) + __logf(l_run);
 }
@@ -176,36 +177,36 @@
 extern "C" __global__ void __launch_bounds__(FF_THREADS, 2)
 fa_fwd_bf16(const unsigned short* q, const unsigned short* k,
             const unsigned short* v, unsigned short* out, float* lse,
-            int B, int Hq, int Hkv, int S, float scale) {
-  fa_fwd_t<0>(q, k, v, out, lse, B, Hq, Hkv, S, scale);
+            int B, int Hq, int Hkv, int S, float scale, int out_bshd) {
+  fa_fwd_t<0>(q, k, v, out, lse, B, Hq, Hkv, S, scale, out_bshd);
 }
 extern "C" __global__ void __launch_bounds__(FF_THREADS, 2)
 fa_fwd_bf16_ab1(const unsigned short* q, const unsigned short* k,
                 const unsigned short* v, unsigned short* out, float* lse,
-                int B, int Hq, int Hkv, int S, float scale) {
-  fa_fwd_t<1>(q, k, v, out, lse, B, Hq, Hkv, S, scale);
+                int B, int Hq, int Hkv, int S, float scale, int out_bshd) {
+  fa_fwd_t<1>(q, k, v, out, lse, B, Hq, Hkv, S, scale, out_bshd);
 }
 extern "C" __global__ void __launch_bounds__(FF_THREADS, 2)
 fa_fwd_bf16_ab2(const unsigned short* q, const unsigned short* k,
                 const unsigned short* v, unsigned short* out, float* lse,
-                int B, int Hq, int Hkv, int S, float scale) {
-  fa_fwd_t<2>(q, k, v, out, lse, B, Hq, Hkv, S, scale);
+                int B, int Hq, int Hkv, int S, float scale, int out_bshd) {
+  fa_fwd_t<2>(q, k, v, out, lse, B, Hq, Hkv, S, scale, out_bshd);
 }
 extern "C" __global__ void __launch_bounds__(FF_THREADS, 2)
 fa_fwd_bf16_ab3(const unsigned short* q, const unsigned short* k,
                 const unsigned short* v, unsigned short* out, float* lse,
-                int B, int Hq, int Hkv, int S, float scale) {
-  fa_fwd_t<3>(q, k, v, out, lse, B, Hq, Hkv, S, scale);
+                int B, int Hq, int Hkv, int S, float scale, int out_bshd) {
+  fa_fwd_t<3>(q, k, v, out, lse, B, Hq, Hkv, S, scale, out_bshd);
 }
 extern "C" __global__ void __launch_bounds__(FF_THREADS, 2)
 fa_fwd_bf16_ab4(const unsigned short* q, const unsigned short* k,
                 const unsigned short* v, unsigned short* out, float* lse,
-                int B, int Hq, int Hkv, int S, float scale) {
-  fa_fwd_t<4>(q, k, v, out, lse, B, Hq, Hkv, S, scale);
+                int B, int Hq, int Hkv, int S, float scale, int out_bshd) {
+  fa_fwd_t<4>(q, k, v, out, lse, B, Hq, Hkv, S, scale, out_bshd);
 }
 extern "C" __global__ void __launch_bounds__(FF_THREADS, 2)
 fa_fwd_bf16_ab5(const unsigned short* q, const unsigned short* k,
                 const unsigned short* v, unsigned short* out, float* lse,
-                int B, int Hq, int Hkv, int S, float scale) {
-  fa_fwd_t<5>(q, k, v, out, lse, B, Hq, Hkv, S, scale);
-}
+                int B, int Hq, int Hkv, int S, float scale, int out_bshd) {
+  fa_fwd_t<5>(q, k, v, out, lse, B, Hq, Hkv, S, scale, out_bshd);
+}
diff --git a/vescale_amd/ops/csrc/extension.hip b/vescale_amd/ops/csrc/extension.hip
--- a/vescale_amd/ops/csrc/extension.hip
+++ b/vescale_amd/ops/csrc/extension.hip
@@ -160,7 +160,9 @@
   if (rows == 0) return {dx, at::zeros({hidden}, x.options().dtype(F32))};
   int grid = (int)std::min<int64_t>(rows, 1024);
   auto dw_part = at::empty({grid, hidden}, x.options().dtype(F32));
-  b.launch(rmsnorm_bwd_bf16, grid, 256, bf16(dy), bf16(x), bf16(w),
+  decltype(&rmsnorm_bwd_bf16) kerns[] = {rmsnorm_bwd_it1_bf16, rmsnorm_bwd_it2_bf16,
+                                         rmsnorm_bwd_it3_bf16, rmsnorm_bwd_bf16};
+  b.launch(kerns[(hidden - 1) / 2048], grid, 256, bf16(dy), bf16(x), bf16(w),
            rrms.data_ptr<float>(), bf16(dres), bf16_mut(dx), dw_part.data_ptr<float>(),
            rows, hidden);
   return {dx, dw_part.sum(0)};
@@ -210,6 +212,14 @@
   return B * S * (Hq + 2 * Hkv) * (D / 2);
 }
 
+bool rope_qkv_v8(int64_t D, std::initializer_list<const at::Tensor*> ts) {
+  if (D % 16 != 0 || D / 16 > 64) return false;
+  for (const at::Tensor* t : ts)
+    if (reinterpret_cast<uintptr_t>(t->const_data_ptr()) % 16 != 0) return false;
+  return true;
+}
+int rope_qkv_v8_grid(int64_t tokens) { return grid_for(tokens, 4, 1 << 16); }
+
 std::vector<at::Tensor> rope_qkv_fwd(at::Tensor qkv, at::Tensor table, int64_t B,
                                      int64_t S, int64_t Hq, int64_t Hkv, int64_t D,
                                      int64_t pos_offset) {
@@ -221,7 +231,10 @@
   auto q = at::empty({B, Hq, S, D}, opt);
   auto k = at::empty({B, Hkv, S, D}, opt);
   auto v = at::empty({B, Hkv, S, D}, opt);
-  b.launch(rope_qkv_fwd_bf16, grid_for(total, 256), 256, bf16(qkv), bf16_mut(q),
+  if (total == 0) return {q, k, v};
+  const bool v8 = rope_qkv_v8(D, {&qkv, &q, &k, &v, &table});
+  b.launch(v8 ? rope_qkv_fwd_v8_bf16 : rope_qkv_fwd_bf16,
+           v8 ? rope_qkv_v8_grid(B * S) : grid_for(total, 256), 256, bf16(qkv), bf16_mut(q),
            bf16_mut(k), bf16_mut(v), table.data_ptr<float>(), B * S, (int)S, (int)Hq,
            (int)Hkv, (int)D, (int)pos_offset);
   return {q, k, v};
@@ -237,9 +250,12 @@
   b.arg("dv", dv, BF16, {B, Hkv, S, D});
   b.arg("table", table, F32, {-1, D / 2, 2});
   auto dqkv = at::empty({B, S, (Hq + 2 * Hkv) * D}, dq.options());
-  b.launch(rope_qkv_bwd_bf16, grid_for(total, 256), 256, bf16(dq), bf16(dk), bf16(dv),
-           bf16_mut(dqkv), table.data_ptr<float>(), B * S, (int)S, (int)Hq, (int)Hkv,
-           (int)D, (int)pos_offset);
+  if (total == 0) return dqkv;
+  const bool v8 = rope_qkv_v8(D, {&dq, &dk, &dv, &dqkv, &table});
+  b.launch(v8 ? rope_qkv_bwd_v8_bf16 : rope_qkv_bwd_bf16,
+           v8 ? rope_qkv_v8_grid(B * S) : grid_for(total, 256), 256, bf16(dq), bf16(dk),
+           bf16(dv), bf16_mut(dqkv), table.data_ptr<float>(), B * S, (int)S, (int)Hq,
+           (int)Hkv, (int)D, (int)pos_offset);
   return dqkv;
 }
 
@@ -457,7 +473,7 @@
 
 FaShape fa_check(const Binding& b, int tile, const at::Tensor& q, const at::Tensor& k,
                  const at::Tensor& v, const OptTensor& o = {},
-                 const OptTensor& dout = {}, const OptTensor& lse = {}) {
+                 const OptTensor& dout = {}, const OptTensor& lse = {}, bool bshd = false) {
   TORCH_CHECK(q.dim() == 4 && k.dim() == 4, b.fn, ": q, k must be [B,H,S,128], got q sizes=",
               q.sizes(), " k sizes=", k.sizes());
   int64_t B = q.size(0), Hq = q.size(1), S = q.size(2), Hkv = k.size(1);
@@ -468,42 +484,50 @@
   b.arg("q", q, BF16, {B, Hq, S, FF_D});
   b.arg("k", k, BF16, {B, Hkv, S, FF_D});
   b.arg("v", v, BF16, {B, Hkv, S, FF_D});
-  b.arg("o", o, BF16, {B, Hq, S, FF_D});
-  b.arg("dout", dout, BF16, {B, Hq, S, FF_D});
+  TORCH_CHECK(!bshd || (B * Hq * S <= INT_MAX && Hq * FF_D * 256 <= INT_MAX), b.fn,
+              ": B * Hq * S and Hq * 32768 must fit int in the [B,S,Hq,D] layout");
+  const Shape oshape = bshd ? Shape{B, S, Hq, FF_D} : Shape{B, Hq, S, FF_D};
+  b.arg("o", o, BF16, oshape);
+  b.arg("dout", dout, BF16, oshape);
   b.arg("lse", lse, F32, {B, Hq, S});
   return {(int)B, (int)Hq, (int)Hkv, (int)S};
 }
 static_assert(FA_D == FF_D && FB_D == FF_D, "tuned attention kernels share D");
 
 std::vector<at::Tensor> fa_fwd_impl(const Binding& b, int64_t mode, at::Tensor q,
-                                    at::Tensor k, at::Tensor v, double scale) {
+                                    at::Tensor k, at::Tensor v, double scale,
+                                    bool out_bshd) {
   FaShape s = fa_check(b, FF_QTILE, q, k, v);
-  auto out = at::empty_like(q);
+  TORCH_CHECK(!out_bshd || (int64_t)s.Hq * FF_D <= INT_MAX, b.fn,
+              ": Hq * 128 must fit int in the [B,S,Hq,D] layout");
+  auto out = out_bshd ? at::empty({s.B, s.S, s.Hq, FF_D}, q.options()) : at::empty_like(q);
   auto lse = at::empty({s.B, s.Hq, s.S}, q.options().dtype(F32));
   decltype(&fa_fwd_bf16) kerns[] = {fa_fwd_bf16,     fa_fwd_bf16_ab1, fa_fwd_bf16_ab2,
                                     fa_fwd_bf16_ab3, fa_fwd_bf16_ab4, fa_fwd_bf16_ab5};
   b.launch(kerns[mode], dim3(s.S / FF_QTILE, s.Hq, s.B), FF_THREADS, bf16(q), bf16(k), bf16(v),
-           bf16_mut(out), lse.data_ptr<float>(), s.B, s.Hq, s.Hkv, s.S, (float)scale);
+           bf16_mut(out), lse.data_ptr<float>(), s.B, s.Hq, s.Hkv, s.S, (float)scale,
+           out_bshd ? 1 : 0);
   return {out, lse};
 }
 
-std::vector<at::Tensor> fa_fwd(at::Tensor q, at::Tensor k, at::Tensor v, double scale) {
-  return fa_fwd_impl(Binding("fa_fwd", "q", q), 0, q, k, v, scale);
+std::vector<at::Tensor> fa_fwd(at::Tensor q, at::Tensor k, at::Tensor v, double scale,
+                               bool out_bshd) {
+  return fa_fwd_impl(Binding("fa_fwd", "q", q), 0, q, k, v, scale, out_bshd);
 }
 
 std::vector<at::Tensor> fa_fwd_ablate(at::Tensor q, at::Tensor k, at::Tensor v,
                                       double scale, int64_t mode) {
   TORCH_CHECK(mode >= 0 && mode <= 5, "fa_fwd_ablate: mode = ", mode,
               " must be in 0..5");
-  return fa_fwd_impl(Binding("fa_fwd_ablate", "q", q), mode, q, k, v, scale);
+  return fa_fwd_impl(Binding("fa_fwd_ablate", "q", q), mode, q, k, v, scale, false);
 }
 
 at::Tensor fa_bwd_delta(const Binding& b, const FaShape& s, const at::Tensor& dout,
-                        const at::Tensor& o) {
+                        const at::Tensor& o, bool bshd = false) {
   auto delta = at::empty({s.B, s.Hq, s.S}, o.options().dtype(F32));
   int64_t rows = (int64_t)s.B * s.Hq * s.S;
   b.launch(fa_bwd_preprocess, grid_for(rows, 1, 4096), 256, bf16(dout), bf16(o),
-           delta.data_ptr<float>(), rows);
+           delta.data_ptr<float>(), rows, s.Hq, s.S, bshd ? 1 : 0);
   return delta;
 }
 
@@ -536,15 +560,17 @@
 
 std::vector<at::Tensor> fa_bwd2(at::Tensor q, at::Tensor k, at::Tensor v, at::Tensor o,
                                 at::Tensor dout, at::Tensor lse, double scale,
-                                bool fused_dvdk) {
+                                bool fused_dvdk, bool bshd) {
   Binding b("fa_bwd2", "q", q);
-  FaShape s = fa_check(b, FB_TILE, q, k, v, o, dout, lse);
-  auto delta = fa_bwd_delta(b, s, dout, o);
+  TORCH_CHECK(!(bshd && fused_dvdk), "fa_bwd2: the fused dv+dk kernel reads [B,Hq,S,D] ",
+              "only: bshd=True needs fused_dvdk=False");
+  FaShape s = fa_check(b, FB_TILE, q, k, v, o, dout, lse, bshd);
+  auto delta = fa_bwd_delta(b, s, dout, o, bshd);
   auto dq = at::empty_like(q);
   dim3 grid(s.S / FB_TILE, s.Hq, s.B);
   b.launch(fa2_dq_bf16, grid, FB_THREADS, bf16(q), bf16(k), bf16(v), bf16(dout),
            lse.data_ptr<float>(), delta.data_ptr<float>(), bf16_mut(dq), s.B, s.Hq,
-           s.Hkv, s.S, (float)scale);
+           s.Hkv, s.S, (float)scale, bshd ? 1 : 0);
   auto dv_part = at::empty_like(q);
   auto dk_part = at::empty_like(q);
   if (fused_dvdk) {
@@ -555,10 +581,10 @@
   } else {
     b.launch(fa2_dv_bf16, grid, FB_THREADS, bf16(q), bf16(k), bf16(dout),
              lse.data_ptr<float>(), bf16_mut(dv_part), s.B, s.Hq, s.Hkv, s.S,
-             (float)scale);
+             (float)scale, bshd ? 1 : 0);
     b.launch(fa2_dk_bf16, grid, FB_THREADS, bf16(q), bf16(k), bf16(v), bf16(dout),
              lse.data_ptr<float>(), delta.data_ptr<float>(), bf16_mut(dk_part), s.B,
-             s.Hq, s.Hkv, s.S, (float)scale);
+             s.Hq, s.Hkv, s.S, (float)scale, bshd ? 1 : 0);
   }
   return {dq, fa_bwd_reduce(b, s, dk_part), fa_bwd_reduce(b, s, dv_part)};
 }
@@ -722,8 +748,11 @@
   m.def("gemm_tn", &gemm_tn, pybind11::arg("a"), pybind11::arg("b"), pybind11::arg("variant") = 0);
   m.def("gemm_tn8", &gemm_tn8, pybind11::arg("a"), pybind11::arg("b"), pybind11::arg("mode") = 0);
   m.def("fa_bwd", &fa_bwd);
-  m.def("fa_bwd2", &fa_bwd2);
-  m.def("fa_fwd", &fa_fwd);
+  m.def("fa_bwd2", &fa_bwd2, pybind11::arg("q"), pybind11::arg("k"), pybind11::arg("v"),
+        pybind11::arg("o"), pybind11::arg("dout"), pybind11::arg("lse"),
+        pybind11::arg("scale"), pybind11::arg("fused_dvdk"), pybind11::arg("bshd") = false);
+  m.def("fa_fwd", &fa_fwd, pybind11::arg("q"), pybind11::arg("k"), pybind11::arg("v"),
+        pybind11::arg("scale"), pybind11::arg("out_bshd") = false);
   m.def("fa_fwd_ablate", &fa_fwd_ablate);
   m.def("fa_gen_fwd", &fa_gen_fwd, pybind11::arg("q"), pybind11::arg("k"),
         pybind11::arg("v"), pybind11::arg("scale"), pybind11::arg("causal"),
diff --git a/vescale_amd/ops/csrc/fa32_common.h b/vescale_amd/ops/csrc/fa32_common.h
--- a/vescale_amd/ops/csrc/fa32_common.h
+++ b/vescale_amd/ops/csrc/fa32_common.h
@@ -75,6 +75,28 @@
   for (int j = 0; j < FF_STAGE_CHUNKS(ROWS, THREADS); ++j) {
     const int e = ff_chunk<THREADS>(j, tid);
     ff_chunk_store(ff_chunk_load(g, e), l, e);
+  }
+}
+
+struct ff_rows {
+  int64_t base;
+  int stride;
+};
+DEV ff_rows ff_o_rows(const ff_ctx& c, int Hq, int S, int bshd) {
+  ff_rows r;
+  r.stride = bshd ? Hq * FF_D : FF_D;
+  r.base = bshd ? ((int64_t)c.b * S * Hq + c.h) * FF_D : c.qbase;
+  return r;
+}
+
+template <int ROWS, int THREADS>
+DEV void ff_stage_rows(const unsigned short* __restrict__ g, int stride, unsigned short* l,
+                       int tid) {
+#pragma unroll
+  for (int j = 0; j < FF_STAGE_CHUNKS(ROWS, THREADS); ++j) {
+    const int e = ff_chunk<THREADS>(j, tid);
+    const int ge = (e / FF_D) * stride + (e % FF_D);
+    ff_chunk_store(ff_chunk_load(g, ge), l, e);
   }
 }
 
diff --git a/vescale_amd/ops/csrc/rmsnorm.hip b/vescale_amd/ops/csrc/rmsnorm.hip
--- a/vescale_amd/ops/csrc/rmsnorm.hip
+++ b/vescale_amd/ops/csrc/rmsnorm.hip
@@ -111,8 +111,8 @@
   }
 }
 
-extern "C" __global__ void __launch_bounds__(BLOCK)
-rmsnorm_bwd_bf16(const unsigned short* __restrict__ dy,
+template <int ITERS>
+DEV void rmsnorm_bwd_t(const unsigned short* __restrict__ dy,
                  const unsigned short* __restrict__ x,
                  const unsigned short* __restrict__ w,
                  const float* __restrict__ rrms_in,
@@ -122,13 +122,12 @@
                  int64_t n_rows, int hidden) {
   __shared__ float lds[BLOCK / WAVE];
   const int vec = 8;
-  const int per_row_iters = (hidden / vec + BLOCK - 1) / BLOCK;
-  float dw_acc[32];
-#pragma unroll
-  for (int j = 0; j < 32; ++j) dw_acc[j] = 0.f;
-  float wreg[32];
+  float dw_acc[ITERS * 8];
+#pragma unroll
+  for (int j = 0; j < ITERS * 8; ++j) dw_acc[j] = 0.f;
+  float wreg[ITERS * 8];
   #pragma unroll
-  for (int it = 0; it < 4; ++it) {
+  for (int it = 0; it < ITERS; ++it) {
     int i = (it * BLOCK + threadIdx.x) * vec;
     if (i < hidden) {
       short8v wv = *reinterpret_cast<const short8v*>(w + i);
@@ -143,9 +142,9 @@
     unsigned short* dxr = dx + row * hidden;
     float rrms = rrms_in[row];
     float dot = 0.f;
-    float dyreg[32], xreg[32];
-#pragma unroll
-    for (int it = 0; it < 4; ++it) {
+    float dyreg[ITERS * 8], xreg[ITERS * 8];
+#pragma unroll
+    for (int it = 0; it < ITERS; ++it) {
       int i = (it * BLOCK + threadIdx.x) * vec;
       if (i < hidden) {
         short8v dv = *reinterpret_cast<const short8v*>(dyr + i);
@@ -163,7 +162,7 @@
     float tdot = block_reduce_sum<BLOCK>(dot, lds);
     float coef = tdot * rrms * rrms * rrms / (float)hidden;
 #pragma unroll
-    for (int it = 0; it < 4; ++it) {
+    for (int it = 0; it < ITERS; ++it) {
       int i = (it * BLOCK + threadIdx.x) * vec;
       if (i < hidden) {
         short8v o;
@@ -185,7 +184,7 @@
   }
   float* dwr = dw_part + (int64_t)blockIdx.x * hidden;
   #pragma unroll
-  for (int it = 0; it < 4; ++it) {
+  for (int it = 0; it < ITERS; ++it) {
     int i = (it * BLOCK + threadIdx.x) * vec;
     if (i < hidden) {
 #pragma unroll
@@ -193,3 +192,16 @@
     }
   }
 }
+
+#define RMSNORM_BWD(NAME, ITERS)                                                \
+  extern "C" __global__ void __launch_bounds__(BLOCK) NAME(                     \
+      const unsigned short* __restrict__ dy, const unsigned short* __restrict__ x, \
+      const unsigned short* __restrict__ w, const float* __restrict__ rrms_in,  \
+      const unsigned short* __restrict__ dres, unsigned short* __restrict__ dx, \
+      float* __restrict__ dw_part, int64_t n_rows, int hidden) {                \
+    rmsnorm_bwd_t<ITERS>(dy, x, w, rrms_in, dres, dx, dw_part, n_rows, hidden); \
+  }
+RMSNORM_BWD(rmsnorm_bwd_bf16, 4)
+RMSNORM_BWD(rmsnorm_bwd_it3_bf16, 3)
+RMSNORM_BWD(rmsnorm_bwd_it2_bf16, 2)
+RMSNORM_BWD(rmsnorm_bwd_it1_bf16, 1)
diff --git a/vescale_amd/ops/csrc/rope_qkv.hip b/vescale_amd/ops/csrc/rope_qkv.hip
--- a/vescale_amd/ops/csrc/rope_qkv.hip
+++ b/vescale_amd/ops/csrc/rope_qkv.hip
@@ -1,4 +1,6 @@
 #include "common.h"
+
+#include <type_traits>
 
 #define BLOCK 256
 
@@ -93,3 +95,103 @@
     }
   }
 }
+
+template <bool BWD>
+DEV void rope_qkv_v8_t(
+    std::conditional_t<BWD, unsigned short, const unsigned short>* __restrict__ packed,
+    std::conditional_t<BWD, const unsigned short, unsigned short>* __restrict__ q,
+    std::conditional_t<BWD, const unsigned short, unsigned short>* __restrict__ k,
+    std::conditional_t<BWD, const unsigned short, unsigned short>* __restrict__ v,
+    const float* __restrict__ table, int64_t n_tokens, int seq, int Hq, int Hkv, int D,
+    int pos_offset) {
+  const int rot = D / 2;
+  const int upd = D / 16;
+  const int slots = WAVE / upd;
+  const int lane = threadIdx.x & (WAVE - 1);
+  const int slot = lane / upd;
+  const int d0 = (lane - slot * upd) * 8;
+  const int heads_total = Hq + 2 * Hkv;
+  const int row = heads_total * D;
+  const int64_t head_stride = (int64_t)seq * D;
+  const int waves = BLOCK / WAVE;
+  if (slot >= slots) return;
+  for (int64_t tok = (int64_t)blockIdx.x * waves + (threadIdx.x / WAVE); tok < n_tokens;
+       tok += (int64_t)gridDim.x * waves) {
+    const int64_t b = tok / seq;
+    const int s = (int)(tok - b * seq);
+    const float4v* tb = reinterpret_cast<const float4v*>(
+        table + ((int64_t)(s + pos_offset) * rot + d0) * 2);
+    float cs[16];
+#pragma unroll
+    for (int j = 0; j < 4; ++j) {
+      float4v t = tb[j];
+#pragma unroll
+      for (int e = 0; e < 4; ++e) cs[j * 4 + e] = t[e];
+    }
+    auto* pk = packed + tok * row + d0;
+    const int64_t in_head = (int64_t)s * D + d0;
+    auto* qt = q + b * Hq * head_stride + in_head;
+    auto* kt = k + b * Hkv * head_stride + in_head;
+    auto* vt = v + b * Hkv * head_stride + in_head;
+#pragma unroll 2
+    for (int h = slot; h < heads_total; h += slots) {
+      const bool roped = h < Hq + Hkv;
+      auto* hp = h < Hq ? qt + h * head_stride
+                        : (roped ? kt + (h - Hq) * head_stride
+                                 : vt + (h - Hq - Hkv) * head_stride);
+      auto* pp = pk + h * D;
+      short8v lo, hi;
+      if constexpr (BWD) {
+        lo = *reinterpret_cast<const short8v*>(hp);
+        hi = *reinterpret_cast<const short8v*>(hp + rot);
+      } else {
+        lo = *reinterpret_cast<const short8v*>(pp);
+        hi = *reinterpret_cast<const short8v*>(pp + rot);
+      }
+      if (roped) {
+#pragma unroll
+        for (int e = 0; e < 8; ++e) {
+          float x0 = bf16_to_f32((unsigned short)lo[e]);
+          float x1 = bf16_to_f32((unsigned short)hi[e]);
+          const float c = cs[2 * e], sn = cs[2 * e + 1];
+          if constexpr (BWD) {
+            lo[e] = (short)f32_to_bf16(__builtin_fmaf(x1, sn, x0 * c));
+            hi[e] = (short)f32_to_bf16(__builtin_fmaf(x1, c, -(x0 * sn)));
+          } else {
+            lo[e] = (short)f32_to_bf16(__builtin_fmaf(x0, c, -(x1 * sn)));
+            hi[e] = (short)f32_to_bf16(__builtin_fmaf(x0, sn, x1 * c));
+          }
+        }
+      }
+      if constexpr (BWD) {
+        *reinterpret_cast<short8v*>(pp) = lo;
+        *reinterpret_cast<short8v*>(pp + rot) = hi;
+      } else {
+        *reinterpret_cast<short8v*>(hp) = lo;
+        *reinterpret_cast<short8v*>(hp + rot) = hi;
+      }
+    }
+  }
+}
+
+extern "C" __global__ void __launch_bounds__(BLOCK)
+rope_qkv_fwd_v8_bf16(const unsigned short* __restrict__ qkv,
+                     unsigned short* __restrict__ q,
+                     unsigned short* __restrict__ k,
+                     unsigned short* __restrict__ v,
+                     const float* __restrict__ table,
+                     int64_t n_tokens, int seq, int Hq, int Hkv, int D,
+                     int pos_offset) {
+  rope_qkv_v8_t<false>(qkv, q, k, v, table, n_tokens, seq, Hq, Hkv, D, pos_offset);
+}
+
+extern "C" __global__ void __launch_bounds__(BLOCK)
+rope_qkv_bwd_v8_bf16(const unsigned short* __restrict__ dq,
+                     const unsigned short* __restrict__ dk,
+                     const unsigned short* __restrict__ dv,
+                     unsigned short* __restrict__ dqkv,
+                     const float* __restrict__ table,
+                     int64_t n_tokens, int seq, int Hq, int Hkv, int D,
+                     int pos_offset) {
+  rope_qkv_v8_t<true>(dqkv, dq, dk, dv, table, n_tokens, seq, Hq, Hkv, D, pos_offset);
+}
diff --git a/vescale_amd/ops/functional.py b/vescale_amd/ops/functional.py
--- a/vescale_amd/ops/functional.py
+++ b/vescale_amd/ops/functional.py
@@ -455,18 +455,24 @@
 
     @staticmethod
     def forward(ctx, q, k, v, scale):
-        out, lse = _ext().fa_fwd(q, k, v, scale)
+        out, lse = _ext().fa_fwd(q, k, v, scale, out_bshd=True)
         ctx.save_for_backward(q, k, v, out, lse)
         ctx.scale = scale
-        return out
+        return out.transpose(1, 2)
 
     @staticmethod
     def backward(ctx, dout):
         q, k, v, out, lse = ctx.saved_tensors
         fused = os.environ.get("VESCALE_FA_FUSED_DVDK", "0") == "1"
-        dq, dk, dv = _ext().fa_bwd2(
-            q, k, v, out, dout.contiguous(), lse, ctx.scale, fused
-        )
+        if fused:
+            dq, dk, dv = _ext().fa_bwd2(
+                q, k, v, out.transpose(1, 2).contiguous(), dout.contiguous(), lse,
+                ctx.scale, True)
+            return dq, dk, dv, None
+        dout = dout.transpose(1, 2)
+        if not dout.is_contiguous():
+            dout = dout.contiguous()
+        dq, dk, dv = _ext().fa_bwd2(q, k, v, out, dout, lse, ctx.scale, False, bshd=True)
         return dq, dk, dv, None
 
 
```

Result: faster. 18480 tokens/s (median of 6 runs) (+2.3%).
